# yetanotherco/yet-another-halo2-fork

Hardware: AMD Instinct MI355X
Metric: create_proof wall-seconds at k=22 (BN254/KZG); MSM Mscalar-mul/s at 2^24 (lower is better)
Workload: dtype u32 limbs (BN254 Fr/Fq Montgomery, 256-bit modular integer)

## Files before the change

include/h2g.h:

```cpp
#ifndef H2G_H
#define H2G_H

#include <stddef.h>
#include <stdint.h>

#ifdef __cplusplus
extern "C" {
#endif

enum {
  H2G_OK = 0,
  H2G_ERR_ARG = 1,
  H2G_ERR_DEVICE = 2,
  H2G_ERR_NOMEM = 3,
  H2G_ERR_STATE = 4,
  H2G_ERR_HANDLE = 5,
  H2G_ERR_UNSATISFIED = 6
};

int h2g_abi_version(void);
const char* h2g_last_error(void);

int h2g_init(const int* devices, int ndev);
int h2g_shutdown(void);
// ... 183 lines not shown
int h2g_params_downsize(uint64_t params, uint32_t k, uint64_t* handle);

int h2g_params_write(uint64_t params, int format, uint8_t* out, size_t cap, size_t* len);
int h2g_params_read(const uint8_t* buf, size_t len, int format, uint64_t* handle);

int h2g_keygen(uint64_t params, const h2g_circuit* circuit, uint64_t* pk);
int h2g_pk_free(uint64_t pk);
int h2g_pk_write(uint64_t pk, int format, uint8_t* out, size_t cap, size_t* len);
int h2g_pk_read(uint64_t params, const h2g_circuit* circuit, const uint8_t* buf, size_t len, int format,
                uint64_t* pk);
enum { H2G_COSETS_RESIDENT = 0, H2G_COSETS_STREAMED = 1 };
typedef struct { uint32_t size; uint32_t cosets; } h2g_key_options;
int h2g_keygen_opts(uint64_t params, const h2g_circuit* circuit, const h2g_key_options* opts, uint64_t* pk);
int h2g_pk_read_opts(uint64_t params, const h2g_circuit* circuit, const uint8_t* buf, size_t len, int format,
                     const h2g_key_options* opts, uint64_t* pk);
int h2g_pk_memory(uint64_t pk, uint64_t out[4]);
int h2g_pk_info(uint64_t pk, int32_t info[8]);
int h2g_pk_lookup_sort_hints(uint64_t pk, int32_t* out, int max, int* count);
int h2g_pk_vk_commitments(uint64_t pk, uint64_t* fixed, uint64_t* perm);
int h2g_pk_set_multiopen(uint64_t pk, int scheme);
int h2g_pk_set_transcript(uint64_t pk, int kind);

int h2g_create_proof(uint64_t params, uint64_t pk, const uint64_t* advice, int advice_on_device,
                     const uint64_t* instance, const uint32_t* instance_lens, const uint8_t rng_seed[32],
                     uint32_t vanishing_threads, uint8_t* proof, size_t proof_cap, size_t* proof_len);
typedef struct {
  void* ctx;
  int (*fill)(void* ctx, uint32_t phase, const uint64_t* challenges, uint64_t* advice);
} h2g_witness_source;
int h2g_create_proof_phased(uint64_t params, uint64_t pk, const h2g_witness_source* witness,
                            const uint64_t* instance, const uint32_t* instance_lens, const uint8_t rng_seed[32],
                            uint32_t vanishing_threads, uint8_t* proof, size_t proof_cap, size_t* proof_len);
typedef struct {
  void* ctx;
  int (*fill_bytes)(void* ctx, uint8_t* out, size_t len);
  int (*random_fr)(void* ctx, uint64_t out[4]);
} h2g_rng;
typedef struct {
  void* ctx;
  int (*fill)(void* ctx, uint32_t circuit, uint32_t phase, const uint64_t* challenges, uint64_t* advice);
} h2g_witness_source_multi;
typedef struct {
  uint32_t num_circuits;
  const uint64_t* const* advice;
  int advice_on_device;
  const h2g_witness_source_multi* witness;
  const uint64_t* const* instance;
  const uint32_t* const* instance_lens;
  const h2g_rng* rng;
  const uint8_t* rng_seed;
  uint32_t vanishing_threads;
} h2g_prove_inputs;
int h2g_create_proof_multi(uint64_t params, uint64_t pk, const h2g_prove_inputs* in, uint8_t* proof,
                           size_t proof_cap, size_t* proof_len);
typedef struct { const uint64_t* index; const uint64_t* den; size_t count; } h2g_assigned_dens;
typedef struct {
  void* ctx;
  int (*fill)(void* ctx, uint32_t circuit, uint32_t phase, const uint64_t* challenges, uint64_t* advice,
              h2g_assigned_dens* dens);
} h2g_assigned_source;
int h2g_create_proof_assigned(uint64_t params, uint64_t pk, const h2g_prove_inputs* in,
                              const h2g_assigned_source* source, uint8_t* proof, size_t proof_cap, size_t* proof_len);
int h2g_rng_chacha20(const uint8_t seed[32], h2g_rng* out, uint64_t* handle);
int h2g_rng_free(uint64_t handle);
int h2g_last_challenges(uint64_t* out, int max, int* count);
enum {
  H2G_CHECK_GATE = 1,
  H2G_CHECK_GATE_BLINDING = 2,
  H2G_CHECK_LOOKUP = 3,
  H2G_CHECK_SHUFFLE = 4,
  H2G_CHECK_COPY = 5
};
#define H2G_CHECK_NO_ROW 0xFFFFFFFFu
typedef struct {
  uint32_t kind, index, row, reserved;
} h2g_check_failure;
typedef struct {
  const uint64_t* advice;
  int advice_on_device;
  const uint64_t* instance;
  const uint64_t* challenges;
  const uint8_t* seed;
  const int32_t* copies;
  uint32_t num_copies;
} h2g_check_inputs;
int h2g_check_witness(uint64_t pk, const h2g_check_inputs* in, h2g_check_failure* out, size_t cap, uint64_t* total);

enum { H2G_SELFCHECK_OFF = 0, H2G_SELFCHECK_VERDICT = 1, H2G_SELFCHECK_ARGUMENTS = 2 };
enum {
  H2G_CHECK_PERMUTATION = 6,
  H2G_CHECK_PRODUCT = 7,
  H2G_CHECK_PERMUTED_PAIR = 8,
  H2G_CHECK_UNUSABLE_ROW = 9,
  H2G_CHECK_IDENTITY = 10
};
int h2g_pk_set_self_check(uint64_t pk, int mode);
int h2g_last_self_check(h2g_check_failure* out, size_t cap, uint64_t* total);
int h2g_debug_selfcheck_product_dev(const void* d_z, const void* d_num_a, const void* d_num_b, const void* d_den_a,
                                    const void* d_den_b, const uint64_t beta[4], const uint64_t gamma[4], uint64_t n,
                                    uint64_t u, int max_blocks, h2g_check_failure* out, size_t cap, uint64_t* total);
int h2g_debug_selfcheck_permuted_dev(const void* d_a, const void* d_s, uint64_t u, int max_blocks,
                                     h2g_check_failure* out, size_t cap, uint64_t* total);
int h2g_debug_selfcheck_permutation_dev(const void* d_z, const uint64_t* first, const void* const* d_values,
                                        const void* const* d_sigmas, const uint64_t* delta_pows, int m,
                                        const uint64_t beta[4], const uint64_t gamma[4], const uint64_t omega[4],
                                        uint64_t u, h2g_check_failure* out, size_t cap, uint64_t* total);

int h2g_vk_from_pk(uint64_t pk, uint64_t* vk);
int h2g_vk_read(const h2g_circuit* circuit, const uint8_t* buf, size_t len, int format, uint64_t* vk);
int h2g_vk_write(uint64_t vk, int format, uint8_t* out, size_t cap, size_t* len);
int h2g_vk_free(uint64_t vk);
typedef struct { uint64_t g1[8], g2[16], s_g2[16]; } h2g_verifier_params;
int h2g_params_verifier(uint64_t params, h2g_verifier_params* out);
typedef struct {
  const uint8_t* proof; size_t proof_len;
  uint32_t num_circuits;
  const uint64_t* const* instance;
  const uint32_t* const* instance_lens;
} h2g_verify_item;
enum { H2G_VERIFY_OK = 1, H2G_VERIFY_REJECTED = 0, H2G_VERIFY_MALFORMED = -1 };
int h2g_verify_proof(uint64_t vk, const h2g_verifier_params* vp, int multiopen, int transcript,
                     const h2g_verify_item* item, int32_t* verdict);
int h2g_verify_batch(uint64_t vk, const h2g_verifier_params* vp, int multiopen, int transcript,
                     const h2g_verify_item* items, size_t count, const h2g_rng* rng,
                     int32_t* verdicts, uint64_t stats[4]);
int h2g_verify_stages(double ms[4]);

int h2g_transcript_new_write(int kind, uint64_t* t);
int h2g_transcript_new_read(int kind, const uint8_t* proof, size_t len, uint64_t* t);
int h2g_transcript_common_point(uint64_t t, const uint64_t p[8]);
int h2g_transcript_common_scalar(uint64_t t, const uint64_t s[4]);
int h2g_transcript_write_point(uint64_t t, const uint64_t p[8]);
int h2g_transcript_write_scalar(uint64_t t, const uint64_t s[4]);
int h2g_transcript_read_point(uint64_t t, uint64_t p[8]);
int h2g_transcript_read_scalar(uint64_t t, uint64_t s[4]);
int h2g_transcript_squeeze(uint64_t t, uint64_t c[4]);
int h2g_transcript_bytes(uint64_t t, uint8_t* out, size_t cap, size_t* len);
int h2g_transcript_remaining(uint64_t t, size_t* bytes);
int h2g_transcript_free(uint64_t t);

int h2g_params_commit(uint64_t params, const uint64_t* coeffs, size_t len, uint64_t out[8], int* is_identity);
int h2g_params_commit_lagrange(uint64_t params, const uint64_t* evals, size_t len, uint64_t out[8], int* is_identity);
int h2g_params_commit_dev(uint64_t params, const void* d_coeffs, size_t len, uint64_t out[8], int* is_identity,
                          void* stream);
int h2g_params_commit_lagrange_dev(uint64_t params, const void* d_evals, size_t len, uint64_t out[8],
                                   int* is_identity, void* stream);
int h2g_fr_eval(const uint64_t* poly, size_t len, const uint64_t x[4], uint64_t out[4]);
int h2g_fr_eval_dev(const void* d_poly, size_t len, const uint64_t x[4], uint64_t out[4], void* stream);
int h2g_kate_division(const uint64_t* a, size_t len, const uint64_t b[4], uint64_t* q);
int h2g_kate_division_dev(const void* d_a, size_t len, const uint64_t b[4], void* d_q, void* stream);
int h2g_debug_kate_division_dev(const void* d_a, size_t len, const uint64_t b[4], void* d_q, int accumulate,
                                int tile_s, void* stream);
int h2g_debug_kate_tile_s(size_t len, int* tile_s);

typedef struct { const uint64_t* coeffs; size_t len; int on_device; } h2g_poly_ref;
typedef struct { uint32_t poly; uint32_t reserved; uint64_t point[4]; } h2g_open_query;
int h2g_multiopen_prove(uint64_t params, int scheme, uint64_t transcript, const h2g_poly_ref* polys, size_t npolys,
                        const h2g_open_query* queries, size_t nqueries);
typedef struct { uint32_t commitment; uint32_t reserved; uint64_t point[4]; uint64_t eval[4]; } h2g_verify_query;
int h2g_multiopen_verify(const h2g_verifier_params* vp, int scheme, uint64_t transcript,
                         const uint64_t* commitments, size_t ncommitments,
                         const h2g_verify_query* queries, size_t nqueries, int32_t* verdict, uint64_t lr[16]);

int h2g_pairing_check_batch(const h2g_verifier_params* vp, const uint64_t* lr, size_t count, int32_t* ok);
int h2g_pairing_check_batch_dev(const h2g_verifier_params* vp, const void* d_lr, size_t count,
                                void* d_ok , void* stream);
int h2g_verify_set_isolation(int mode);
int h2g_debug_pairing_values(const h2g_verifier_params* vp, const uint64_t* lr, size_t count,
                             uint64_t* miller, uint64_t* gt);

int h2g_prover_stage_sync(int on);
int h2g_prover_stages(double* ms, int max, int* count);
const char* h2g_prover_stage_name(int i);

typedef struct {
  void* ctx;
  int32_t world;
  int (*launch)(void* ctx, uint64_t seq, int32_t base_set, uint64_t n, const void* d_scalars);
  int (*collect)(void* ctx, uint64_t seq, uint64_t* partials, int32_t* is_identity);
} h2g_shard_transport;
int h2g_set_shard_transport(const h2g_shard_transport* t);
int h2g_params_set_slab(uint64_t params, uint64_t lo, uint64_t hi);
int h2g_params_msm_dev(uint64_t params, int32_t base_set, uint64_t offset, uint64_t n, const void* d_scalars,
                       uint64_t out_affine[8], int32_t* out_is_identity);
int h2g_params_table_bytes(uint64_t params, uint64_t out[4]);
int h2g_memcpy_dtod(void* d_dst, const void* d_src, size_t bytes);

int h2g_comm_unique_id(uint8_t id[256]);
int h2g_comm_init(const uint8_t id[256], int world, int rank);
int h2g_comm_set_timeout(double seconds);
int h2g_comm_set_serve_timeout(double seconds);
int h2g_comm_keepalive(void);
int h2g_comm_install(uint64_t params);
int h2g_comm_serve(uint64_t params, uint64_t* served);
int h2g_comm_stop(void);
int h2g_comm_destroy(void);
int h2g_comm_info(int32_t* rccl_count, int32_t* rccl_rank);

#define H2G_SPMD_WORDS 13
typedef struct {
  void* ctx;
  int32_t world;
  int32_t rank;
  int (*allgather)(void* ctx, uint64_t seq, const uint64_t in[9], uint64_t* out);
  int (*bcast)(void* ctx, void* d_buf, size_t bytes, int root);
  int (*allgather_host)(void* ctx, const void* in, size_t bytes, void* out);
  int (*exchange)(void* ctx, const void* d_send, const size_t* send_bytes, void* d_recv, const size_t* recv_bytes);
} h2g_spmd_transport;
int h2g_set_spmd_transport(const h2g_spmd_transport* t);
typedef int (*h2g_spmd_exchange_post)(void* ctx, const void* d_send, const size_t* send_bytes, void* d_recv,
                                      const size_t* recv_bytes, void* stream, void* done);
typedef int (*h2g_spmd_exchange_wait)(void* ctx, void* done);
int h2g_set_spmd_exchange_async(h2g_spmd_exchange_post post, h2g_spmd_exchange_wait wait);
int h2g_event_wait(void* done);
int h2g_debug_link_delay(void* stream, void* done, double us);
int h2g_spmd_set_weights(const uint32_t* weights, int world);
int h2g_spmd_set_column_owners(int on);
int h2g_spmd_stats(double* out, int max, int reset);
int h2g_comm_spmd_install(int split_subcosets);
int h2g_comm_set_exchange_overlap(int on);
int h2g_comm_spmd_uninstall(void);

#ifdef __cplusplus
}
#endif

#endif
```

yet-another-halo2-fork_amd/csrc/keygen.cpp:

```cpp
#include "prover_state.h"

using namespace h2g;
using namespace h2g::rt;
using namespace h2g::prv;

namespace {
struct CircuitView {
  const h2g_circuit* c;
  const int32_t* node(int i) const { return c->nodes + 4 * i; }
};

int node_degree(const CircuitView& v, int i, std::vector<int>& memo) {
  if (memo[i] >= 0) return memo[i];
  const int32_t* nd = v.node(i);
  int d = 0;
  switch (nd[0]) {
    case OP_CONST:
    case OP_CHALLENGE: d = 0; break;
    case OP_QUERY: d = 1; break;
    case OP_NEG: d = node_degree(v, nd[1], memo); break;
    case OP_SUM: d = std::max(node_degree(v, nd[1], memo), node_degree(v, nd[2], memo)); break;
    default: d = node_degree(v, nd[1], memo) + node_degree(v, nd[2], memo); break;
  }
  return memo[i] = d;
// ... 263 lines not shown
  HIPCHK(hipMemcpy(w->d_perm_v, pv.data(), pv.size() * sizeof(Fr*), hipMemcpyHostToDevice));
  pk.cws.push_back(std::move(w));
  return H2G_OK;
}

int key_options_mode(const h2g_key_options* opts, const char* who, int* mode) {
  *mode = H2G_COSETS_RESIDENT;
  if (!opts) return H2G_OK;
  if (opts->size < sizeof(h2g_key_options)) return fail(H2G_ERR_ARG, std::string(who) + ": key options: bad size");
  if (opts->cosets != H2G_COSETS_RESIDENT && opts->cosets != H2G_COSETS_STREAMED)
    return fail(H2G_ERR_ARG, std::string(who) + ": key options: unknown coset mode");
  *mode = (int)opts->cosets;
  return H2G_OK;
}

int build_pow_table(Pool& pool, const Fr& w, int L, PowTable* t, hipStream_t st) {
  const int bits = (L + 1) / 2;
  const size_t nlo = (size_t)1 << bits, nhi = (size_t)1 << (L - bits > 0 ? L - bits : 0);
  std::vector<Fr> lo(nlo), hi(nhi);
  lo[0] = Fr::one();
  for (size_t i = 1; i < nlo; i++) lo[i] = lo[i - 1] * w;
  const Fr wb = lo[nlo - 1] * w;
  hi[0] = Fr::one();
  for (size_t i = 1; i < nhi; i++) hi[i] = hi[i - 1] * wb;
  Fr *dlo, *dhi;
  PALLOC(pool, dlo, nlo);
  PALLOC(pool, dhi, nhi);
  HIPCHK(hipMemcpyAsync(dlo, lo.data(), nlo * sizeof(Fr), hipMemcpyHostToDevice, st));
  HIPCHK(hipMemcpyAsync(dhi, hi.data(), nhi * sizeof(Fr), hipMemcpyHostToDevice, st));
  HIPCHK(hipStreamSynchronize(st));
  t->lo = dlo;
  t->hi = dhi;
  t->bits = bits;
  return H2G_OK;
}

int cs_host_build(const h2g_circuit* c, CsHost* out) {
  CsHost& cs = *out;
  cs = CsHost{};
  std::string why;
  if (c->num_gates && (!c->gate_roots || !c->nodes)) return fail(H2G_ERR_ARG, "keygen: null gates");
  if (!check_nodes(c, &why)) return fail(H2G_ERR_ARG, "keygen: bad expression graph: " + why);
  if (!c->transcript_repr) return fail(H2G_ERR_ARG, "keygen: null transcript_repr");
  if (c->k > FR_S) return fail(H2G_ERR_ARG, "keygen: k too large");
  const CircuitView cv{c};
  const size_t n = (size_t)1 << c->k;
  cs.k = c->k;
  cs.A = (int)c->num_advice;
  cs.F = (int)c->num_fixed;
  cs.I = (int)c->num_instance;
  cs.P = (int)c->num_perm_columns;
  cs.transcript_repr = fr_from_limbs(c->transcript_repr);
  cs.adv_phase.assign(cs.A, 0);
  if (c->advice_phase)
    for (int i = 0; i < cs.A; i++) cs.adv_phase[i] = c->advice_phase[i];
  cs.ch_phase.assign(c->num_challenges, 0);
  if (c->num_challenges && !c->challenge_phase) return fail(H2G_ERR_ARG, "keygen: null challenge_phase");
  for (uint32_t i = 0; i < c->num_challenges; i++) cs.ch_phase[i] = c->challenge_phase[i];
  cs.max_phase = 0;
  for (int i = 0; i < cs.A; i++) cs.max_phase = std::max(cs.max_phase, (int)cs.adv_phase[i]);
  for (uint8_t ph : cs.ch_phase)
    if ((int)ph > cs.max_phase) return fail(H2G_ERR_ARG, "keygen: challenge phase after the last advice phase");
  if (cs.P && !c->perm_columns) return fail(H2G_ERR_ARG, "keygen: null permutation columns");
  for (int i = 0; i < cs.P; i++) {
    const int t = c->perm_columns[2 * i], ix = c->perm_columns[2 * i + 1];
    const int lim = t == COL_ADVICE ? cs.A : t == COL_FIXED ? cs.F : t == COL_INSTANCE ? cs.I : 0;
    if (ix < 0 || ix >= lim) return fail(H2G_ERR_ARG, "keygen: permutation column out of range");
    cs.perm_cols.emplace_back(t, ix);
  }
  std::vector<int> memo(c->num_nodes, -1);
  const std::vector<ArgRoots> lks = arg_roots(c->num_lookups, c->lookup_sizes, c->lookup_roots);
  const std::vector<ArgRoots> shs = arg_roots(c->num_shuffles, c->shuffle_sizes, c->shuffle_roots);
  cs.NL = (int)lks.size();
  cs.NS = (int)shs.size();
  cs.degree = 3;
  for (uint32_t g = 0; g < c->num_gates; g++) cs.degree = std::max(cs.degree, node_degree(cv, c->gate_roots[g], memo));
  for (const auto& a : lks) {
    int di = 1, dt = 1;
    for (int i = 0; i < a.m; i++) {
      di = std::max(di, node_degree(cv, a.in[i], memo));
      dt = std::max(dt, node_degree(cv, a.other[i], memo));
    }
    cs.degree = std::max(cs.degree, std::max(4, 2 + di + dt));
  }
  for (const auto& a : shs) {
    int di = 1, ds = 1;
    for (int i = 0; i < a.m; i++) {
      di = std::max(di, node_degree(cv, a.in[i], memo));
      ds = std::max(ds, node_degree(cv, a.other[i], memo));
    }
    cs.degree = std::max(cs.degree, 2 + std::max(di, ds));
  }
  for (uint32_t g = 0; g < c->num_gates; g++) collect(cv, c->gate_roots[g], cs);
  for (const auto& a : lks) {
    for (int i = 0; i < a.m; i++) collect(cv, a.in[i], cs);
    for (int i = 0; i < a.m; i++) collect(cv, a.other[i], cs);
  }
  for (const auto& a : shs) {
    for (int i = 0; i < a.m; i++) collect(cv, a.in[i], cs);
    for (int i = 0; i < a.m; i++) collect(cv, a.other[i], cs);
  }
  for (auto& pc : cs.perm_cols)
    add_query(pc.first == COL_ADVICE ? cs.adv_q : (pc.first == COL_FIXED ? cs.fix_q : cs.ins_q),
              Query{pc.first, pc.second, 0});
  int maxq = 1;
  if (cs.A) {
    std::vector<int> cnt(cs.A, 0);
    for (auto& q : cs.adv_q) cnt[q.index]++;
    maxq = *std::max_element(cnt.begin(), cnt.end());
  }
  cs.bf = std::max(3, maxq) + 2;
  if ((int64_t)n < cs.bf + 3) return fail(H2G_ERR_ARG, "keygen: not enough rows available");
  cs.chunk_len = cs.degree - 2;
  cs.nsets = (cs.P + cs.chunk_len - 1) / cs.chunk_len;
  if (c->num_nodes) cs.nodes.assign(c->nodes, c->nodes + 4 * (size_t)c->num_nodes);
  if (c->num_constants && !c->constants) return fail(H2G_ERR_ARG, "keygen: null constants");
  cs.constants.resize(c->num_constants);
  for (uint32_t i = 0; i < c->num_constants; i++) cs.constants[i] = fr_from_limbs(c->constants + 4 * i);
  if (c->num_gates) cs.gate_roots.assign(c->gate_roots, c->gate_roots + c->num_gates);
  for (const auto& a : lks) {
    cs.lk_in.emplace_back(a.in, a.in + a.m);
    cs.lk_tab.emplace_back(a.other, a.other + a.m);
  }
  for (const auto& a : shs) {
    cs.sh_in.emplace_back(a.in, a.in + a.m);
    cs.sh_sh.emplace_back(a.other, a.other + a.m);
  }
  return H2G_OK;
}

int keygen_impl(Device* d, Params& prm, const h2g_circuit* c, ProvingKey& pk, const PkImage* img = nullptr) {
  hipStream_t st = d->stream;
  if (c->k != prm.k) return fail(H2G_ERR_ARG, "keygen: circuit k != params k");
  RCCHK(cs_host_build(c, &pk.cs));
  if (!img && c->num_fixed && !c->fixed_values) return fail(H2G_ERR_ARG, "keygen: null fixed values");
  const CircuitView cv{c};
  const std::vector<ArgRoots> lks = arg_roots(c->num_lookups, c->lookup_sizes, c->lookup_roots);
  const std::vector<ArgRoots> shs = arg_roots(c->num_shuffles, c->shuffle_sizes, c->shuffle_roots);
  pk.device = d->id;
  pk.n = (size_t)1 << pk.cs.k;
  pk.unblinded.assign(pk.cs.A, 0);
  if (c->unblinded)
    for (int i = 0; i < pk.cs.A; i++) pk.unblinded[i] = c->unblinded[i];
  pk.num_consts = (int)c->num_constants;
  RCCHK(domain_init(&pk.dom, (uint32_t)pk.cs.degree, pk.cs.k));
  pk.ext = (size_t)1 << pk.dom.ek;
  pk.rot_scale = 1ull << (pk.dom.ek - pk.cs.k);
  const size_t n = pk.n, ext = pk.ext;
  Pool& pool = pk.pool;
  RCCHK(build_pow_table(pool, pk.dom.omega, (int)pk.cs.k, &pk.om, st));
  RCCHK(build_pow_table(pool, pk.dom.ext_omega, (int)pk.dom.ek, &pk.eo, st));

  auto falloc = [&](Fr** p, size_t cnt) { return pool.get((void**)p, cnt * sizeof(Fr)); };
  pk.scr_len = std::max(n + 64, kate_scratch_len(n) + poly_prefix_scratch_len(n) + 64);
  HIPCHK(falloc(&pk.mod, n));
  HIPCHK(falloc(&pk.pre, n));
  HIPCHK(falloc(&pk.scr, pk.scr_len));
  HIPCHK(falloc(&pk.random_poly, n));
  HIPCHK(falloc(&pk.h_ext, ext));
  HIPCHK(falloc(&pk.h_coeff, ext));
  HIPCHK(falloc(&pk.h_poly, n));
  HIPCHK(falloc(&pk.nx, n));
  HIPCHK(falloc(&pk.q1, n));
  HIPCHK(falloc(&pk.hx, n));
  HIPCHK(falloc(&pk.lx, n));
  HIPCHK(falloc(&pk.small, 4096));
  HIPCHK(falloc(&pk.last_z, 1));
  auto vec_alloc = [&](std::vector<Fr*>& v, int cnt, size_t len) -> hipError_t {
    v.assign(cnt, nullptr);
    for (int i = 0; i < cnt; i++) {
      hipError_t e = falloc(&v[i], len);
      if (e != hipSuccess) return e;
    }
    return hipSuccess;
  };
  HIPCHK(falloc(&pk.one, 1));
  {
    const Fr one = Fr::one();
    HIPCHK(hipMemcpy(pk.one, &one, sizeof(Fr), hipMemcpyHostToDevice));
  }
  if (pk.cs.NL + pk.cs.NS) {
    HIPCHK(falloc(&pk.tmp_a, n));
    HIPCHK(falloc(&pk.tmp_b, n));
  }
  if (pk.cs.NL) {
    PALLOC(pool, pk.ck_a2, n);
    PALLOC(pool, pk.ck_t2, n);
    PALLOC(pool, pk.ck_left, n);
    PALLOC(pool, pk.rep_flag, n);
    PALLOC(pool, pk.left_flag, n);
    PALLOC(pool, pk.rep_rows, n);
    PALLOC(pool, pk.counters, 8);
    pk.lk_hb.assign(pk.cs.NL, 64);
  }

  const bool streamed = pk.cosets != 0;
  const size_t clen = streamed ? n : ext;
  auto image_coset = [&](Fr* resident, const uint8_t* src) -> int {
    Fr* dst = streamed ? pk.h_ext : resident;
    HIPCHK(img->upload(dst, src, ext, st));
    if (streamed && img->bad_raw) HIPCHK(fr_count_unreduced(dst, ext, img->bad_raw, st));
    return H2G_OK;
  };
  if (streamed) HIPCHK(falloc(&pk.h_gather, ext));
  HIPCHK(vec_alloc(pk.fixed_lag, pk.cs.F, n));
  HIPCHK(vec_alloc(pk.fixed_poly, pk.cs.F, n));
  HIPCHK(vec_alloc(pk.fixed_coset, pk.cs.F, clen));
  for (int i = 0; i < pk.cs.F; i++) {
    if (img) {
      HIPCHK(img->upload(pk.fixed_lag[i], img->fixed_lag[i], n, st));
      HIPCHK(img->upload(pk.fixed_poly[i], img->fixed_poly[i], n, st));
      RCCHK(image_coset(pk.fixed_coset[i], img->fixed_coset[i]));
      continue;
    }
    HIPCHK(hipMemcpyAsync(pk.fixed_lag[i], c->fixed_values + 4 * n * i, n * sizeof(Fr), hipMemcpyHostToDevice, st));
    RCCHK(lagrange_to_coeff(d, pk.dom, pk.fixed_lag[i], pk.fixed_poly[i], st));
    if (!streamed) RCCHK(coeff_to_extended(d, pk.dom, pk.fixed_poly[i], pk.fixed_coset[i], st));
  }
  HIPCHK(falloc(&pk.l0, clen));
  HIPCHK(falloc(&pk.l_last, clen));
  HIPCHK(falloc(&pk.l_active, clen));
  if (img) {
    RCCHK(image_coset(pk.l0, img->l0));
    RCCHK(image_coset(pk.l_last, img->l_last));
    RCCHK(image_coset(pk.l_active, img->l_active));
  }
  if (!img || streamed) {
    const Fr one = Fr::one();
    std::vector<Fr> ones(pk.cs.bf, one);
    auto lagrange_unit = [&](size_t row0, int count, Fr* poly, Fr* out) -> int {
      HIPCHK(hipMemsetAsync(pk.pre, 0, n * sizeof(Fr), st));
      HIPCHK(hipMemcpyAsync(pk.pre + row0, ones.data(), count * sizeof(Fr), hipMemcpyHostToDevice, st));
      RCCHK(lagrange_to_coeff(d, pk.dom, pk.pre, poly, st));
      if (out) RCCHK(coeff_to_extended(d, pk.dom, poly, out, st));
      HIPCHK(hipStreamSynchronize(st));
      return H2G_OK;
    };
    if (streamed) {
      HIPCHK(falloc(&pk.l0_poly, n));
      HIPCHK(falloc(&pk.l_last_poly, n));
      HIPCHK(falloc(&pk.l_blind_poly, n));
      RCCHK(lagrange_unit(0, 1, pk.l0_poly, nullptr));
      RCCHK(lagrange_unit(n - pk.cs.bf, pk.cs.bf, pk.l_blind_poly, nullptr));
      RCCHK(lagrange_unit(n - pk.cs.bf - 1, 1, pk.l_last_poly, nullptr));
    } else {
      RCCHK(lagrange_unit(0, 1, pk.mod, pk.l0));
      RCCHK(lagrange_unit(n - pk.cs.bf, pk.cs.bf, pk.mod, pk.h_ext));
      RCCHK(lagrange_unit(n - pk.cs.bf - 1, 1, pk.mod, pk.l_last));
      HIPCHK(poly_binop(POLY_ADD, pk.l_last, pk.h_ext, one, pk.l_active, ext, st));
      HIPCHK(poly_binop(POLY_SUB_CONST, pk.l_active, nullptr, one, pk.l_active, ext, st));
      HIPCHK(poly_binop(POLY_SCALE, pk.l_active, nullptr, fr_neg_one(), pk.l_active, ext, st));
    }
  }
  HIPCHK(vec_alloc(pk.sigma_lag, pk.cs.P, n));
  HIPCHK(vec_alloc(pk.sigma_poly, pk.cs.P, n));
  HIPCHK(vec_alloc(pk.sigma_coset, pk.cs.P, clen));
  if (pk.cs.P && img) {
    for (int i = 0; i < pk.cs.P; i++) {
      HIPCHK(img->upload(pk.sigma_lag[i], img->sigma_lag[i], n, st));
      HIPCHK(img->upload(pk.sigma_poly[i], img->sigma_poly[i], n, st));
      RCCHK(image_coset(pk.sigma_coset[i], img->sigma_coset[i]));
    }
    HIPCHK(hipStreamSynchronize(st));
  } else if (pk.cs.P) {
    const size_t cells = (size_t)pk.cs.P * n;
    std::vector<uint32_t> mcol(cells), mrow(cells), acol(cells), arow(cells);
    std::vector<uint64_t> sizes(cells, 1);
    for (int cI = 0; cI < pk.cs.P; cI++)
      for (size_t r = 0; r < n; r++) {
        mcol[cI * n + r] = acol[cI * n + r] = (uint32_t)cI;
        mrow[cI * n + r] = arow[cI * n + r] = (uint32_t)r;
      }
    auto pos = [&](int t, int ix) -> int {
      for (int i = 0; i < pk.cs.P; i++)
        if (pk.cs.perm_cols[i].first == t && pk.cs.perm_cols[i].second == ix) return i;
      return -1;
    };
    for (uint32_t ci = 0; ci < c->num_copies; ci++) {
      const int32_t* cp = c->copies + 6 * ci;
      const int lc = pos(cp[0], cp[1]), rc = pos(cp[3], cp[4]);
      if (lc < 0 || rc < 0) return fail(H2G_ERR_ARG, "keygen: copy on a column not in the permutation");
      if (cp[2] < 0 || cp[5] < 0 || (size_t)cp[2] >= n || (size_t)cp[5] >= n)
        return fail(H2G_ERR_ARG, "keygen: copy row out of bounds");
      const size_t li = lc * n + cp[2], ri = rc * n + cp[5];
      size_t lcyc = acol[li] * n + arow[li], rcyc = acol[ri] * n + arow[ri];
      if (lcyc == rcyc) continue;
      if (sizes[lcyc] < sizes[rcyc]) std::swap(lcyc, rcyc);
      sizes[lcyc] += sizes[rcyc];
      size_t i = rcyc;
      for (;;) {
        acol[i] = (uint32_t)(lcyc / n);
        arow[i] = (uint32_t)(lcyc % n);
        i = (size_t)mcol[i] * n + mrow[i];
        if (i == rcyc) break;
      }
      std::swap(mcol[li], mcol[ri]);
      std::swap(mrow[li], mrow[ri]);
    }
    std::vector<Fr> dpow(pk.cs.P + 1);
    dpow[0] = Fr::one();
    for (int i = 1; i <= pk.cs.P; i++) dpow[i] = dpow[i - 1] * fr_delta();
    uint32_t *dmc, *dmr;
    Fr* ddp;
    HIPCHK(hipMalloc(&dmc, cells * 4));
    HIPCHK(hipMalloc(&dmr, cells * 4));
    HIPCHK(hipMalloc(&ddp, dpow.size() * sizeof(Fr)));
    HIPCHK(hipMemcpyAsync(dmc, mcol.data(), cells * 4, hipMemcpyHostToDevice, st));
// ... 194 lines not shown
```

yet-another-halo2-fork_amd/csrc/kzg.cpp:

```cpp
#include "multiopen.h"

using namespace h2g;
using namespace h2g::rt;
using namespace h2g::prv;

namespace h2g {
namespace prv {
std::map<uint64_t, std::unique_ptr<TranscriptObj>> g_transcripts;

bool TranscriptObj::read_point(G1Affine* out) {
  if (!read || bytes.size() - pos < 32) return false;
  G1Affine p;
  if (!g1_from_bytes_host(bytes.data() + pos, &p) || p.is_identity()) return false;
  if (!tr.common_point(p)) return false;
  pos += 32;
  *out = p;
  return true;
}
bool TranscriptObj::read_scalar(Fr* out) {
  if (!read || bytes.size() - pos < 32) return false;
  Fr c;
  std::memcpy(c.l, bytes.data() + pos, 32);
  unsigned br = 0;
  for (int i = 0; i < 8; i++) (void)__builtin_subc(c.l[i], FrParams::M[i], br, &br);
// ... 87 lines not shown
  if (len) obj->bytes.assign(proof, proof + len);
  *t = g_next_handle++;
  g_transcripts[*t] = std::move(obj);
  return H2G_OK;
}
int h2g_transcript_free(uint64_t t) {
  std::lock_guard<std::recursive_mutex> lk(g_mu);
  if (!g_transcripts.erase(t)) return fail(H2G_ERR_HANDLE, "unknown transcript");
  return H2G_OK;
}
int h2g_transcript_common_point(uint64_t t, const uint64_t p[8]) {
  NEED_TRANSCRIPT(t);
  G1Affine a;
  if (!p || !point_arg(p, &a)) return fail(H2G_ERR_ARG, "transcript: not a point of the curve, or the identity");
  T->tr.common_point(a);
  return H2G_OK;
}
int h2g_transcript_common_scalar(uint64_t t, const uint64_t s[4]) {
  NEED_TRANSCRIPT(t);
  if (!s || !fr_reduced(fr_from_limbs(s))) return fail(H2G_ERR_ARG, "transcript: scalar not below r");
  T->tr.common_scalar(fr_from_limbs(s));
  return H2G_OK;
}
int h2g_transcript_write_point(uint64_t t, const uint64_t p[8]) {
  NEED_TRANSCRIPT(t);
  if (T->read) return fail(H2G_ERR_ARG, "transcript_write_point: a read-mode transcript");
  G1Affine a;
  if (!p || !point_arg(p, &a))
    return fail(H2G_ERR_ARG, "cannot write points at infinity (or off the curve) to the transcript");
  T->tr.write_point(a);
  return H2G_OK;
}
int h2g_transcript_write_scalar(uint64_t t, const uint64_t s[4]) {
  NEED_TRANSCRIPT(t);
  if (T->read) return fail(H2G_ERR_ARG, "transcript_write_scalar: a read-mode transcript");
  if (!s || !fr_reduced(fr_from_limbs(s))) return fail(H2G_ERR_ARG, "transcript: scalar not below r");
  T->tr.write_scalar(fr_from_limbs(s));
  return H2G_OK;
}
int h2g_transcript_read_point(uint64_t t, uint64_t p[8]) {
  NEED_TRANSCRIPT(t);
  if (!T->read) return fail(H2G_ERR_ARG, "transcript_read_point: a write-mode transcript");
  G1Affine a;
  if (!p || !T->read_point(&a))
    return fail(H2G_ERR_ARG, "transcript_read_point: the bytes end, or no valid encoding of a point other than the identity");
  std::memcpy(p, &a, sizeof(G1Affine));
  return H2G_OK;
}
int h2g_transcript_read_scalar(uint64_t t, uint64_t s[4]) {
  NEED_TRANSCRIPT(t);
  if (!T->read) return fail(H2G_ERR_ARG, "transcript_read_scalar: a write-mode transcript");
  Fr v;
  if (!s || !T->read_scalar(&v)) return fail(H2G_ERR_ARG, "transcript_read_scalar: the bytes end, or a value >= r");
  fr_to_limbs(v, s);
  return H2G_OK;
}
int h2g_transcript_squeeze(uint64_t t, uint64_t c[4]) {
  NEED_TRANSCRIPT(t);
  if (!c) return fail(H2G_ERR_ARG, "transcript_squeeze: null argument");
  fr_to_limbs(T->tr.squeeze(), c);
  return H2G_OK;
}
int h2g_transcript_bytes(uint64_t t, uint8_t* out, size_t cap, size_t* len) {
  NEED_TRANSCRIPT(t);
  if (T->read) return fail(H2G_ERR_ARG, "transcript_bytes: a read-mode transcript");
  if (!len) return fail(H2G_ERR_ARG, "transcript_bytes: null argument");
  *len = T->bytes.size();
  if (!out) return H2G_OK;
  if (cap < T->bytes.size()) return fail(H2G_ERR_ARG, "transcript_bytes: buffer too small");
  if (!T->bytes.empty()) std::memcpy(out, T->bytes.data(), T->bytes.size());
  return H2G_OK;
}
int h2g_transcript_remaining(uint64_t t, size_t* bytes) {
  NEED_TRANSCRIPT(t);
  if (!T->read) return fail(H2G_ERR_ARG, "transcript_remaining: a write-mode transcript");
  if (!bytes) return fail(H2G_ERR_ARG, "transcript_remaining: null argument");
  *bytes = T->bytes.size() - T->pos;
  return H2G_OK;
}

int h2g_params_commit(uint64_t params, const uint64_t* coeffs, size_t len, uint64_t out[8], int* is_identity) {
  return commit_entry(params, SRS_G, coeffs, false, len, out, is_identity, nullptr);
}
int h2g_params_commit_lagrange(uint64_t params, const uint64_t* evals, size_t len, uint64_t out[8], int* is_identity) {
  return commit_entry(params, SRS_LAGRANGE, evals, false, len, out, is_identity, nullptr);
}
int h2g_params_commit_dev(uint64_t params, const void* d_coeffs, size_t len, uint64_t out[8], int* is_identity,
                          void* stream) {
  return commit_entry(params, SRS_G, d_coeffs, true, len, out, is_identity, stream);
}
int h2g_params_commit_lagrange_dev(uint64_t params, const void* d_evals, size_t len, uint64_t out[8],
                                   int* is_identity, void* stream) {
  return commit_entry(params, SRS_LAGRANGE, d_evals, true, len, out, is_identity, stream);
}

int h2g_fr_eval_dev(const void* d_poly, size_t len, const uint64_t x[4], uint64_t out[4], void* stream) {
  NEED_DEV_P();
  if (!x || !out || (len && !d_poly)) return fail(H2G_ERR_ARG, "fr_eval: null argument");
  if ((uintptr_t)d_poly % 16) return fail(H2G_ERR_ARG, "fr_eval: the polynomial must be 16-byte aligned");
  if (len == 0) {
    fr_to_limbs(Fr::zero(), out);
    return H2G_OK;
  }
  hipStream_t st = pick_stream(d, stream);
  const size_t scr = poly_eval_scratch_len(1, len);
  HIPCHK(d->work.ensure(128 + scr * sizeof(Fr)));
  uint8_t* w = d->work.as<uint8_t>();
  const EvalReq rq{(const Fr*)d_poly, (uint64_t)len, fr_from_limbs(x)};
  Fr r;
  HIPCHK(hipMemcpyAsync(w, &rq, sizeof(rq), hipMemcpyHostToDevice, st));
  HIPCHK(poly_eval_batch((const EvalReq*)w, 1, len, (Fr*)(w + 64), (Fr*)(w + 128), st));
  HIPCHK(hipMemcpyAsync(&r, w + 64, sizeof(Fr), hipMemcpyDeviceToHost, st));
  HIPCHK(hipStreamSynchronize(st));
  fr_to_limbs(r, out);
  return H2G_OK;
}
int h2g_fr_eval(const uint64_t* poly, size_t len, const uint64_t x[4], uint64_t out[4]) {
  NEED_DEV_P();
  if (len && !poly) return fail(H2G_ERR_ARG, "fr_eval: null argument");
  HIPCHK(d->a.ensure(len * sizeof(Fr) + 32));
  HIPCHK(hipMemcpyAsync(d->a.p, poly, len * sizeof(Fr), hipMemcpyHostToDevice, d->stream));
  return h2g_fr_eval_dev(d->a.p, len, x, out, nullptr);
}
int h2g_kate_division_dev(const void* d_a, size_t len, const uint64_t b[4], void* d_q, void* stream) {
  NEED_DEV_P();
  if (len == 0) return fail(H2G_ERR_ARG, "kate_division: an empty polynomial");
  if (!d_a || !b || (len > 1 && !d_q)) return fail(H2G_ERR_ARG, "kate_division: null argument");
  if ((uintptr_t)d_a % 16 || (uintptr_t)d_q % 16)
    return fail(H2G_ERR_ARG, "kate_division: device arrays must be 16-byte aligned");
  if (len == 1) return H2G_OK;
  HIPCHK(d->work.ensure(kate_scratch_len(len) * sizeof(Fr) + 32));
  HIPCHK(kate_division((const Fr*)d_a, len, fr_from_limbs(b), (Fr*)d_q, d->work.as<Fr>(), pick_stream(d, stream)));
  return H2G_OK;
}
int h2g_debug_kate_division_dev(const void* d_a, size_t len, const uint64_t b[4], void* d_q, int accumulate,
                                int tile_s, void* stream) {
  NEED_DEV_P();
  if (len == 0) return fail(H2G_ERR_ARG, "kate_division: an empty polynomial");
  if (!d_a || !b || (len > 1 && !d_q)) return fail(H2G_ERR_ARG, "kate_division: null argument");
  if ((uintptr_t)d_a % 16 || (uintptr_t)d_q % 16)
    return fail(H2G_ERR_ARG, "kate_division: device arrays must be 16-byte aligned");
  if (tile_s != 0 && tile_s != 8 && tile_s != 16 && tile_s != 32 && tile_s != 64)
    return fail(H2G_ERR_ARG, "debug_kate_division: tile_s must be 0, 8, 16, 32 or 64");
  if (len == 1) return H2G_OK;
  HIPCHK(d->work.ensure(kate_scratch_len(len) * sizeof(Fr) + 32));
  HIPCHK(kate_division((const Fr*)d_a, len, fr_from_limbs(b), (Fr*)d_q, d->work.as<Fr>(), pick_stream(d, stream),
                       accumulate != 0, tile_s));
  return H2G_OK;
}
int h2g_debug_kate_tile_s(size_t len, int* tile_s) {
  if (len == 0) return fail(H2G_ERR_ARG, "kate_division: an empty polynomial");
  if (!tile_s) return fail(H2G_ERR_ARG, "debug_kate_tile_s: null argument");
  *tile_s = kate_tile_s((uint64_t)len - 1);
  return H2G_OK;
}
int h2g_kate_division(const uint64_t* a, size_t len, const uint64_t b[4], uint64_t* q) {
  NEED_DEV_P();
  if (len == 0) return fail(H2G_ERR_ARG, "kate_division: an empty polynomial");
  if (!a || !b || (len > 1 && !q)) return fail(H2G_ERR_ARG, "kate_division: null argument");
  if (len == 1) return H2G_OK;
  HIPCHK(d->a.ensure(len * sizeof(Fr) + 32));
  HIPCHK(d->b.ensure(len * sizeof(Fr) + 32));
  HIPCHK(hipMemcpyAsync(d->a.p, a, len * sizeof(Fr), hipMemcpyHostToDevice, d->stream));
  RCCHK(h2g_kate_division_dev(d->a.p, len, b, d->b.p, nullptr));
  HIPCHK(hipMemcpyAsync(q, d->b.p, (len - 1) * sizeof(Fr), hipMemcpyDeviceToHost, d->stream));
  HIPCHK(hipStreamSynchronize(d->stream));
  return H2G_OK;
}

int h2g_multiopen_prove(uint64_t params, int scheme, uint64_t transcript, const h2g_poly_ref* polys, size_t npolys,
                        const h2g_open_query* queries, size_t nqueries) {
  NEED_DEV_P();
  Params* ip = find_params(params);
  if (!ip) return fail(H2G_ERR_HANDLE, "unknown params");
  TranscriptObj* T = find_transcript(transcript);
  if (!T) return fail(H2G_ERR_HANDLE, "unknown transcript");
  Params& prm = *ip;
  if (prm.device != d->id) return fail(H2G_ERR_ARG, "multiopen_prove: params live on another device");
  if (scheme != MULTIOPEN_SHPLONK && scheme != MULTIOPEN_GWC)
    return fail(H2G_ERR_ARG, "multiopen_prove: scheme must be 0 (SHPLONK) or 1 (GWC)");
  if (T->read) return fail(H2G_ERR_ARG, "multiopen_prove: a read-mode transcript");
  if (!polys || !queries || npolys == 0 || nqueries == 0)
    return fail(H2G_ERR_ARG, "multiopen_prove: no polynomials or no queries");
  if (npolys > (1u << 24) || nqueries > (1u << 24)) return fail(H2G_ERR_ARG, "multiopen_prove: too many queries");
  const size_t n = prm.n;
  if (n < 2) return fail(H2G_ERR_ARG, "multiopen_prove: params of a single point");
  if (g_spmd.world > 1 || g_shard.world > 1)
    return fail(H2G_ERR_STATE, "multiopen_prove: a shard or SPMD transport is installed");
  for (size_t i = 0; i < npolys; i++) {
    const h2g_poly_ref& p = polys[i];
    if (!p.coeffs || p.len == 0) return fail(H2G_ERR_ARG, "multiopen_prove: polynomial " + std::to_string(i) + " is empty");
    if (p.len > n)
      return fail(H2G_ERR_ARG, "multiopen_prove: polynomial " + std::to_string(i) + " is longer than the params' n");
    if (p.on_device && (uintptr_t)p.coeffs % 16)
      return fail(H2G_ERR_ARG, "multiopen_prove: device polynomial " + std::to_string(i) + " is not 16-byte aligned");
  }
  std::vector<OpenQ> qs(nqueries);
  for (size_t i = 0; i < nqueries; i++) {
    if (queries[i].poly >= npolys)
      return fail(H2G_ERR_ARG, "multiopen_prove: query " + std::to_string(i) + " names an unknown polynomial");
    qs[i] = {(int)queries[i].poly, fr_from_limbs(queries[i].point)};
    if (!fr_reduced(qs[i].pt)) return fail(H2G_ERR_ARG, "multiopen_prove: query " + std::to_string(i) + ": point not below r");
  }
  hipStream_t st = d->stream;
  if (!prm.kzg_ws) prm.kzg_ws = std::make_shared<MultiopenWs>();
  MultiopenWs& ws = *static_cast<MultiopenWs*>(prm.kzg_ws.get());
  if (!ws.nx) {
    PALLOC(ws.pool, ws.nx, n);
    PALLOC(ws.pool, ws.hx, n);
    PALLOC(ws.pool, ws.lx, n);
    PALLOC(ws.pool, ws.q1, n);
    PALLOC(ws.pool, ws.scr, kate_scratch_len(n));
  }
  HIPCHK(ws.small.ensure(nqueries + 1));
  Pool call;
  MsmRingGuard ring_guard{d};
  StreamSyncGuard guard{st};
  std::vector<PolyRef> prs(npolys);
  for (size_t i = 0; i < npolys; i++) {
    const h2g_poly_ref& p = polys[i];
    if (p.on_device) {
      prs[i] = {(const Fr*)p.coeffs, (uint64_t)p.len};
      continue;
    }
    Fr* dp;
    PALLOC(call, dp, p.len);
    HIPCHK(hipMemcpyAsync(dp, p.coeffs, p.len * sizeof(Fr), hipMemcpyHostToDevice, st));
    prs[i] = {dp, (uint64_t)p.len};
  }
  std::vector<OpenQ> keys;
  std::vector<std::vector<int>> of(npolys);
  auto index = [&](int poly, const Fr& pt) -> int {
    for (int i : of[poly])
      if (keys[i].pt == pt) return i;
    return -1;
  };
  for (const OpenQ& q : qs)
    if (index(q.poly, q.pt) < 0) {
      keys.push_back(q);
      of[q.poly].push_back((int)keys.size() - 1);
    }
  const int nreq = (int)keys.size();
  std::vector<Fr> evals(nreq);
  {
    uint64_t max_len = 1;
    std::vector<EvalReq> reqs(nreq);
    for (int i = 0; i < nreq; i++) {
      reqs[i] = EvalReq{prs[keys[i].poly].p, prs[keys[i].poly].len, keys[i].pt};
      max_len = std::max<uint64_t>(max_len, reqs[i].len);
    }
    EvalReq* d_reqs;
    Fr *d_out, *d_scr;
    PALLOC(call, d_reqs, nreq);
    PALLOC(call, d_out, nreq);
    PALLOC(call, d_scr, poly_eval_scratch_len(nreq, max_len));
    HIPCHK(hipMemcpyAsync(d_reqs, reqs.data(), nreq * sizeof(EvalReq), hipMemcpyHostToDevice, st));
    HIPCHK(poly_eval_batch(d_reqs, nreq, max_len, d_out, d_scr, st));
    HIPCHK(hipMemcpyAsync(evals.data(), d_out, nreq * sizeof(Fr), hipMemcpyDeviceToHost, st));
    HIPCHK(hipStreamSynchronize(st));
  }
  TranscriptObj run = *T;
  MultiopenCtx c;
  c.d = d;
  c.prm = &prm;
  c.st = st;
  c.tr = &run.tr;
  c.n = n;
  c.polys = &prs;
  c.queries = &qs;
  c.ev = [&](int poly, const Fr& pt) { return evals[index(poly, pt)]; };
  c.nx = ws.nx, c.hx = ws.hx, c.lx = ws.lx, c.q1 = ws.q1, c.scr = ws.scr, c.small = ws.small.p;
  c.gwc_q = &ws.gwc_q;
  c.pool = &ws.pool;
  c.upload = [st](void* dst, const void* src, size_t bytes) {
    return hipMemcpyAsync(dst, src, bytes, hipMemcpyHostToDevice, st);
  };
  c.sl = Slab{0, n, n};
  RCCHK(scheme == MULTIOPEN_GWC ? multiopen_gwc(c) : multiopen_shplonk(c));
  HIPCHK(hipStreamSynchronize(st));
  *T = run;
  return H2G_OK;
}

}
```

yet-another-halo2-fork_amd/csrc/multiopen.cpp:

```cpp
#include "multiopen.h"

using namespace h2g;
using namespace h2g::rt;
using namespace h2g::prv;

namespace {
std::vector<std::vector<Fr>> lagrange_basis(const std::vector<Fr>& pts) {
  const size_t m = pts.size();
  std::vector<std::vector<Fr>> out(m);
  for (size_t j = 0; j < m; j++) {
    std::vector<Fr> num(1, Fr::one());
    Fr den = Fr::one();
    for (size_t k = 0; k < m; k++) {
      if (k == j) continue;
      std::vector<Fr> nn(num.size() + 1, Fr::zero());
      for (size_t i = 0; i < num.size(); i++) {
        nn[i + 1] = nn[i + 1] + num[i];
        nn[i] = nn[i] - pts[k] * num[i];
      }
      num.swap(nn);
      den = den * (pts[j] - pts[k]);
    }
    const Fr sc = inv(den);
    for (Fr& c : num) c = c * sc;
// ... 49 lines not shown
}
void mark(MultiopenCtx& c, const char* name) {
  if (c.mark) c.mark(name);
}
}

namespace h2g {
namespace prv {

int fr_cmp(const Fr& a, const Fr& b) {
  const Fr ca = to_canonical(a), cb = to_canonical(b);
  for (int i = 7; i >= 0; i--) {
    if (ca.l[i] < cb.l[i]) return -1;
    if (ca.l[i] > cb.l[i]) return 1;
  }
  return 0;
}

int multiopen_gwc(MultiopenCtx& c) {
  Transcript& tr = *c.tr;
  const std::vector<PolyRef>& polys = *c.polys;
  const std::vector<OpenQ>& queries = *c.queries;
  const size_t n = c.n;
  hipStream_t st = c.st;
  const Fr v = tr.squeeze();
  std::vector<char> done(queries.size(), 0);
  std::vector<MsmTicket> tk;
  std::vector<Fr> neg_evb;
  neg_evb.reserve(queries.size());
  StreamSyncGuard evb_guard{st};
  for (size_t i = 0; i < queries.size(); i++) {
    if (done[i]) continue;
    const Fr z = queries[i].pt;
    const size_t g = tk.size();
    if (g >= c.gwc_q->size()) {
      Fr* q;
      PALLOC(*c.pool, q, n);
      c.gwc_q->push_back(q);
    }
    LinTerms t;
    bool first = true;
    Fr vp = Fr::one(), evb = Fr::zero();
    for (size_t j = i; j < queries.size(); j++) {
      if (done[j] || queries[j].pt != z) continue;
      done[j] = 1;
      if (t.k == LIN_MAXT - 1) {
        HIPCHK(lincomb(c.nx, n, t, !first, st));
        first = false;
        t.k = 0;
      }
      t.p[t.k] = polys[queries[j].poly].p;
      t.len[t.k] = polys[queries[j].poly].len;
      t.coef[t.k] = vp;
      t.k++;
      evb = evb + vp * c.ev(queries[j].poly, z);
      vp = vp * v;
    }
    neg_evb.push_back(Fr::zero() - evb);
    HIPCHK(c.upload(c.small + g, &neg_evb.back(), sizeof(Fr)));
    t.p[t.k] = c.small + g;
    t.len[t.k] = 1;
    t.coef[t.k] = Fr::one();
    t.k++;
    HIPCHK(lincomb(c.nx, n, t, !first, st));
    HIPCHK(kate_division(c.nx, n, z, (*c.gwc_q)[g], c.scr, st));
    tk.emplace_back();
    RCCHK(commit_launch(c.d, *c.prm, (*c.gwc_q)[g], n - 1, SRS_G, st, &tk.back()));
  }
  {
    std::vector<MsmTicket*> tl;
    for (auto& t : tk) tl.push_back(&t);
    std::vector<G1Affine> cms(tl.size());
    RCCHK(commit_collect_all(c.d, tl.data(), (int)tl.size(), cms.data()));
    for (const G1Affine& cm : cms) RCCHK(write_point(c, cm));
  }
  HIPCHK(hipStreamSynchronize(st));
  mark(c, "gwc");
  return H2G_OK;
}

int multiopen_shplonk(MultiopenCtx& c) {
  Transcript& tr = *c.tr;
  const std::vector<PolyRef>& polys = *c.polys;
  const std::vector<OpenQ>& queries = *c.queries;
  const size_t n = c.n;
  hipStream_t st = c.st;
  const bool slabs = c.slabs;
  const Slab sl = slabs ? c.sl : Slab{0, n, n};
  std::vector<std::vector<Fr>> corr_stage;
  Fr c0_stage;
  StreamSyncGuard corr_guard{st};
  const Fr sy = tr.squeeze();
  std::vector<Fr> super_pts;
  for (auto& q : queries) {
    bool f = false;
    for (auto& p : super_pts) f = f || p == q.pt;
    if (!f) super_pts.push_back(q.pt);
  }
  std::sort(super_pts.begin(), super_pts.end(), [](const Fr& a, const Fr& b) { return fr_cmp(a, b) < 0; });
  std::vector<int> cm_ids;
  std::vector<std::vector<Fr>> cm_pts;
  for (auto& q : queries) {
    int f = -1;
    for (size_t i = 0; i < cm_ids.size(); i++)
      if (cm_ids[i] == q.poly) f = (int)i;
    if (f < 0) {
      f = (int)cm_ids.size();
      cm_ids.push_back(q.poly);
      cm_pts.emplace_back();
    }
    auto& ps = cm_pts[f];
    if (std::find(ps.begin(), ps.end(), q.pt) == ps.end()) ps.push_back(q.pt);
  }
  for (auto& ps : cm_pts) std::sort(ps.begin(), ps.end(), [](const Fr& a, const Fr& b) { return fr_cmp(a, b) < 0; });
  std::vector<int> rs_of(cm_ids.size()), rs_rep;
  for (size_t ci = 0; ci < cm_ids.size(); ci++) {
    int f = -1;
    for (size_t r = 0; r < rs_rep.size(); r++)
      if (cm_pts[rs_rep[r]] == cm_pts[ci]) f = (int)r;
    if (f < 0) {
      f = (int)rs_rep.size();
      rs_rep.push_back((int)ci);
    }
    rs_of[ci] = f;
  }
  std::vector<std::vector<std::vector<Fr>>> basis(rs_rep.size());
  for (size_t r = 0; r < rs_rep.size(); r++) basis[r] = lagrange_basis(cm_pts[rs_rep[r]]);
  std::vector<std::vector<Fr>> low(cm_ids.size());
  for (size_t ci = 0; ci < cm_ids.size(); ci++) {
    const auto& B = basis[rs_of[ci]];
    const size_t m = cm_pts[ci].size();
    low[ci].assign(m, Fr::zero());
    for (size_t j = 0; j < m; j++) {
      const Fr e = c.ev(cm_ids[ci], cm_pts[ci][j]);
      for (size_t i = 0; i < m; i++) low[ci][i] = low[ci][i] + B[j][i] * e;
    }
  }
  const Fr v = tr.squeeze();
  {
    std::vector<Fr> vpow(rs_rep.size()), ypow(cm_ids.size());
    {
      Fr vp = Fr::one();
      for (size_t r = 0; r < rs_rep.size(); r++) {
        vpow[r] = vp;
        vp = vp * v;
        Fr yp = Fr::one();
        for (size_t ci = 0; ci < cm_ids.size(); ci++)
          if (rs_of[ci] == (int)r) {
            ypow[ci] = yp;
            yp = yp * sy;
          }
      }
    }
    const size_t np = super_pts.size(), cap = sl.hi1 - sl.lo + 1;
    if (slabs) HIPCHK(c.slab_pk->slab_buf.ensure(np * cap));
    auto gbuf = [&](size_t i) { return c.slab_pk->slab_buf.p + i * cap - sl.lo; };
    if (slabs) HIPCHK(hipMemsetAsync(c.hx + sl.lo, 0, (sl.hi1 - sl.lo) * sizeof(Fr), st));
    else HIPCHK(hipMemsetAsync(c.hx, 0, n * sizeof(Fr), st));
    for (size_t pi = 0; pi < np; pi++) {
      const Fr& p = super_pts[pi];
      Fr* gp = slabs ? gbuf(pi) : c.nx;
      std::vector<Fr> alpha(rs_rep.size(), Fr::zero());
      std::vector<char> has(rs_rep.size(), 0);
      size_t ncorr = 0;
      for (size_t r = 0; r < rs_rep.size(); r++) {
        const std::vector<Fr>& pts = cm_pts[rs_rep[r]];
        if (std::find(pts.begin(), pts.end(), p) == pts.end()) continue;
        Fr den = Fr::one();
        for (const Fr& q : pts)
          if (!(q == p)) den = den * (p - q);
        alpha[r] = vpow[r] * inv(den);
        has[r] = 1;
        ncorr = std::max(ncorr, pts.size());
      }
      corr_stage.emplace_back(ncorr, Fr::zero());
      std::vector<Fr>& corr = corr_stage.back();
      LinTerms t;
      bool first = true;
      for (size_t ci = 0; ci < cm_ids.size(); ci++) {
        const int r = rs_of[ci];
        if (!has[r]) continue;
        if (t.k == LIN_MAXT - 1) {
          RCCHK(lincomb_range(gp, sl.lo, sl.hi1, t, !first, st));
          first = false;
          t.k = 0;
        }
        const Fr coef = alpha[r] * ypow[ci];
        t.p[t.k] = polys[cm_ids[ci]].p;
        t.len[t.k] = polys[cm_ids[ci]].len;
        t.coef[t.k] = coef;
        t.k++;
        for (size_t j = 0; j < low[ci].size(); j++) corr[j] = corr[j] + coef * low[ci][j];
      }
      HIPCHK(c.upload(c.small, corr.data(), corr.size() * sizeof(Fr)));
      t.p[t.k] = c.small;
      t.len[t.k] = corr.size();
      t.coef[t.k] = fr_neg_one();
      t.k++;
      RCCHK(lincomb_range(gp, sl.lo, sl.hi1, t, !first, st));
      if (!slabs) HIPCHK(kate_division(c.nx, n, p, c.hx, c.scr, st, true));
    }
    if (slabs) {
      std::vector<Fr> carry;
      RCCHK(slab_carries(c, super_pts, [&](size_t i) { return gbuf(i); }, &carry));
      Fr halo = Fr::zero();
      for (size_t pi = 0; pi < np; pi++) {
        const size_t hq = std::min(sl.hi, n - 1);
        if (hq <= sl.lo) continue;
        HIPCHK(poly_binop(POLY_ADD_CONST, gbuf(pi) + hq, nullptr, super_pts[pi] * carry[pi], gbuf(pi) + hq, 1, st));
        HIPCHK(kate_division(gbuf(pi) + sl.lo, hq - sl.lo + 1, super_pts[pi], c.hx + sl.lo, c.scr, st, true));
        halo = halo + carry[pi];
      }
      if (sl.hi < n) {
        corr_stage.emplace_back(1, halo);
        HIPCHK(c.upload(c.hx + sl.hi, corr_stage.back().data(), sizeof(Fr)));
      }
    }
  }
  {
    G1Affine cm;
    RCCHK(commit(c.d, *c.prm, c.hx, n, SRS_G, &cm, st));
    RCCHK(write_point(c, cm));
  }
  mark(c, "shplonk h");
  const Fr u = tr.squeeze();
  Fr z0 = Fr::one();
  {
    Fr vpow = Fr::one(), c0 = Fr::zero();
    LinTerms t;
    bool first = true;
    auto flush = [&]() -> int {
      RCCHK(lincomb_range(c.lx, sl.lo, sl.hi1, t, !first, st));
      first = false;
      t.k = 0;
      return H2G_OK;
    };
    for (size_t r = 0; r < rs_rep.size(); r++) {
      const std::vector<Fr>& pts = cm_pts[rs_rep[r]];
      Fr zi = Fr::one();
      for (auto& sp : super_pts)
        if (std::find(pts.begin(), pts.end(), sp) == pts.end()) zi = (u - sp) * zi;
      if (r == 0) z0 = zi;
      Fr ypow = Fr::one();
      for (size_t ci = 0; ci < cm_ids.size(); ci++) {
        if (rs_of[ci] != (int)r) continue;
        if (t.k == LIN_MAXT - 2) RCCHK(flush());
        const Fr coef = ypow * zi * vpow;
        t.p[t.k] = polys[cm_ids[ci]].p;
        t.len[t.k] = polys[cm_ids[ci]].len;
        t.coef[t.k] = coef;
        t.k++;
        c0 = c0 - coef * eval_host(low[ci], u);
        ypow = ypow * sy;
      }
      vpow = vpow * v;
    }
    Fr zt = Fr::one();
    for (auto& sp : super_pts) zt = (u - sp) * zt;
    c0_stage = c0;
    HIPCHK(c.upload(c.small, &c0_stage, sizeof(Fr)));
    t.p[t.k] = c.small;
    t.len[t.k] = 1;
    t.coef[t.k] = Fr::one();
    t.k++;
    t.p[t.k] = c.hx;
    t.len[t.k] = n;
    t.coef[t.k] = Fr::zero() - zt;
    t.k++;
    RCCHK(flush());
  }
  if (slabs) {
    std::vector<Fr> carry;
    const std::vector<Fr> pts{u};
    RCCHK(slab_carries(c, pts, [&](size_t) { return c.lx; }, &carry));
    const size_t hq = std::min(sl.hi, n - 1);
    if (hq > sl.lo) {
      HIPCHK(poly_binop(POLY_ADD_CONST, c.lx + hq, nullptr, u * carry[0], c.lx + hq, 1, st));
      HIPCHK(kate_division(c.lx + sl.lo, hq - sl.lo + 1, u, c.q1 + sl.lo, c.scr, st));
      HIPCHK(poly_binop(POLY_SCALE, c.q1 + sl.lo, nullptr, inv(z0), c.q1 + sl.lo, hq - sl.lo, st));
    }
  } else {
    HIPCHK(kate_division(c.lx, n, u, c.q1, c.scr, st));
    HIPCHK(poly_binop(POLY_SCALE, c.q1, nullptr, inv(z0), c.q1, n - 1, st));
  }
  {
    G1Affine cm;
    RCCHK(commit(c.d, *c.prm, c.q1, n - 1, SRS_G, &cm, st));
    RCCHK(write_point(c, cm));
  }
  mark(c, "shplonk final");
  return H2G_OK;
}

void msm_merge(Msm& m) {
  std::stable_sort(m.begin(), m.end(), [](const Term& a, const Term& b) { return a.base < b.base; });
  size_t w = 0;
  for (size_t i = 0; i < m.size(); i++) {
    if (w && m[w - 1].base == m[i].base) m[w - 1].s = m[w - 1].s + m[i].s;
    else m[w++] = m[i];
  }
  m.resize(w);
}

bool multiopen_verify_terms(int scheme, const std::vector<VerifierQ>& queries, MultiopenVerifyIo& io, Msm* left_out,
                            Msm* right_out) {
  Transcript& T = *io.T;
  const std::vector<Fr>& point = io.point;
  const Fr one = Fr::one();
  Msm& left = *left_out;
  Msm& right = *right_out;
  if (scheme == MULTIOPEN_GWC) {
    const Fr v = T.squeeze();
    std::vector<int> group_pt;
    std::vector<std::vector<const VerifierQ*>> groups;
    for (const auto& q : queries) {
      size_t g = 0;
      while (g < group_pt.size() && group_pt[g] != q.pt) g++;
      if (g == group_pt.size()) {
        group_pt.push_back(q.pt);
        groups.emplace_back();
      }
      groups[g].push_back(&q);
    }
    if (io.expect_groups >= 0 && groups.size() != (size_t)io.expect_groups) return false;
    std::vector<uint32_t> ws(groups.size());
    for (auto& w : ws) w = io.read_point();
    const Fr u = T.squeeze();
    if (!io.ok()) return false;
    Fr eval_multi = Fr::zero(), upow = one;
    for (size_t g = 0; g < groups.size(); g++) {
      Fr evb = Fr::zero(), vpow = one;
      for (const VerifierQ* q : groups[g]) {
        io.add_obj(right, q->key, vpow * upow);
        evb = evb + vpow * q->eval;
        vpow = vpow * v;
      }
      eval_multi = eval_multi + upow * evb;
      right.push_back({ws[g], upow * point[group_pt[g]]});
      left.push_back({ws[g], upow});
      upow = upow * u;
    }
    right.push_back({BASE_G1, Fr::zero() - eval_multi});
    return true;
  }
  struct Cm {
    uint32_t key;
    std::vector<int> pts;
    std::vector<Fr> evals;
  };
  std::vector<Cm> cms;
  for (const auto& q : queries) {
    size_t i = 0;
    while (i < cms.size() && cms[i].key != q.key) i++;
    if (i == cms.size()) cms.push_back({q.key, {}, {}});
    Cm& cm = cms[i];
    size_t p = 0;
    while (p < cm.pts.size() && cm.pts[p] < q.pt) p++;
    if (p < cm.pts.size() && cm.pts[p] == q.pt) {
      cm.evals[p] = q.eval;
    } else {
      cm.pts.insert(cm.pts.begin() + p, q.pt);
      cm.evals.insert(cm.evals.begin() + p, q.eval);
    }
  }
  std::vector<std::vector<int>> set_pts;
  std::vector<std::vector<const Cm*>> set_cms;
  for (const auto& cm : cms) {
    size_t s = 0;
    while (s < set_pts.size() && set_pts[s] != cm.pts) s++;
    if (s == set_pts.size()) {
      set_pts.push_back(cm.pts);
      set_cms.emplace_back();
    }
    set_cms[s].push_back(&cm);
  }
  std::vector<int> super;
  for (const auto& q : queries)
    if (std::find(super.begin(), super.end(), q.pt) == super.end()) super.push_back(q.pt);
  const Fr sy = T.squeeze();
  const Fr v = T.squeeze();
  const uint32_t h1 = io.read_point();
  const Fr u = T.squeeze();
  const uint32_t h2 = io.read_point();
  if (!io.ok()) return false;
  Fr z0 = Fr::zero(), z0_diff_inv = Fr::zero(), r_outer = Fr::zero(), vpow = one;
  for (size_t s = 0; s < set_pts.size(); s++) {
    const std::vector<int>& pts_s = set_pts[s];
    Fr z_diff = one;
    for (int p : super)
      if (std::find(pts_s.begin(), pts_s.end(), p) == pts_s.end()) z_diff = z_diff * (u - point[p]);
    if (s == 0) {
      z0 = one;
      for (int p : pts_s) z0 = z0 * (u - point[p]);
      z0_diff_inv = inv(z_diff);
      z_diff = one;
    } else {
      z_diff = z_diff * z0_diff_inv;
    }
    std::vector<Fr> basis(pts_s.size());
    for (size_t j = 0; j < pts_s.size(); j++) {
      Fr num = one, den = one;
      for (size_t k = 0; k < pts_s.size(); k++) {
        if (k == j) continue;
        num = num * (u - point[pts_s[k]]);
        den = den * (point[pts_s[j]] - point[pts_s[k]]);
      }
      basis[j] = num * inv(den);
    }
    Fr r_inner = Fr::zero(), ypow = one;
    const Fr scale = vpow * z_diff;
    for (const Cm* cm : set_cms[s]) {
      Fr ru = Fr::zero();
      for (size_t j = 0; j < pts_s.size(); j++) ru = ru + cm->evals[j] * basis[j];
      r_inner = r_inner + ypow * ru;
      io.add_obj(right, cm->key, ypow * scale);
      ypow = ypow * sy;
    }
    r_outer = r_outer + vpow * r_inner * z_diff;
    vpow = vpow * v;
  }
  right.push_back({BASE_G1, Fr::zero() - r_outer});
  right.push_back({h1, Fr::zero() - z0});
  right.push_back({h2, u});
  left.push_back({h2, one});
  return true;
}

}
}
```

yet-another-halo2-fork_amd/csrc/prover_kernels.h:

```cpp
#pragma once
#include "bn254.h"

namespace h2g {

struct PowTable {
  const Fr* lo = nullptr;
  const Fr* hi = nullptr;
  int bits = 0;
};

static constexpr int PERM_MAXC = 8;
struct PermCols {
  const Fr* v[PERM_MAXC];
  const Fr* sigma[PERM_MAXC];
  Fr beta_delta[PERM_MAXC];
  int m = 0;
};
hipError_t perm_denominators(Fr* out, size_t n, const PermCols& c, const Fr& beta, const Fr& gamma, bool init,
                             hipStream_t st);
hipError_t perm_numerators(Fr* mod, size_t n, const PermCols& c, const Fr& gamma, const PowTable& omega,
                           hipStream_t st, size_t r0 = 0);
hipError_t perm_z_assemble(Fr* z, size_t n, int bf, const Fr* prefix, const Fr* last_z, const Fr* blind_rows,
                           hipStream_t st, size_t lo = 0, size_t hi = ~(size_t)0);

// ... 20 lines not shown
  const EvalLookup* lookups = nullptr;
  const EvalShuffle* shuffles = nullptr;
  const Fr* consts = nullptr;
  const Fr* const* query_col = nullptr;
  const int* query_rot = nullptr;
  int nsets = 0, chunk_len = 0, P = 0;
  const Fr* const* z = nullptr;
  const Fr* const* perm_v = nullptr;
  const Fr* const* sigma = nullptr;
  const Fr* l0 = nullptr;
  const Fr* l_last = nullptr;
  const Fr* l_active = nullptr;
  Fr beta, gamma, y, delta_start, delta;
  PowTable ext_omega;
  uint64_t ext = 0, rot_scale = 0;
  uint64_t row0 = 0, rows = 0;
  int last_rot = 0;
  const Fr* t_evals = nullptr;
  uint64_t t_mask = 0;
  const Fr* acc_in = nullptr;
  int divide = 1;
  Fr* out = nullptr;
};
hipError_t evaluate_h(const EvalHArgs& a, hipStream_t st);

hipError_t subcoset_twist(const Fr* src, Fr* dst, size_t n, const PowTable& eo, uint64_t t, uint64_t ext_mask,
                          hipStream_t st);
hipError_t subcoset_gather(const Fr* full, Fr* out, size_t n, uint64_t t, int e, hipStream_t st);
hipError_t subcoset_scatter(const Fr* subs, Fr* ext, size_t n, int e, hipStream_t st);
struct CopySeg {
  const Fr* src;
  Fr* dst;
  uint64_t len;
};
hipError_t copy_segments(const CopySeg* d_segs, int nseg, uint64_t max_len, hipStream_t st);
static constexpr int COPY_COLS_MAX = 16;
struct ColCopy {
  const Fr* src[COPY_COLS_MAX];
  Fr* dst[COPY_COLS_MAX];
  unsigned long long* sum[COPY_COLS_MAX];
};
hipError_t copy_columns(const ColCopy& b, int m, size_t n, bool sums, hipStream_t st);

static constexpr int PREFIX_DIFF_MAX = 16;
struct PrefixDiff {
  const Fr* a[PREFIX_DIFF_MAX];
  Fr* e[PREFIX_DIFF_MAX];
};
hipError_t prefix_diff(const PrefixDiff& b, int m, size_t n, hipStream_t st);
int evaluate_h_max_slots();
static constexpr int HSLAB_MAX_E = 16;
struct HSlabArgs {
  const Fr* recv = nullptr;
  int idx[HSLAB_MAX_E] = {};
  int E = 0, np = 0;
  uint64_t cnt = 0, n = 0, lo = 0;
  const Fr* coef = nullptr;
  Fr* out = nullptr;
};
hipError_t h_slab_combine(const HSlabArgs& a, hipStream_t st);

struct CompressArgs {
  const int4* prog = nullptr;
  int2 seg = {0, 0};
  int n_slots = 0;
  const Fr* consts = nullptr;
  const Fr* const* load_col = nullptr;
  const int* load_rot = nullptr;
  uint64_t n = 0;
  Fr theta;
  Fr* out = nullptr;
};
hipError_t compress_lagrange(const CompressArgs& a, hipStream_t st);
static constexpr int COMPRESS_BATCH_MAX = 32;
struct CompressBatch {
  const int4* prog = nullptr;
  int n_slots = 0;
  const Fr* consts = nullptr;
  const int* load_rot = nullptr;
  uint64_t n = 0;
  Fr theta;
  int count = 0;
  int2 seg[COMPRESS_BATCH_MAX];
  const Fr* const* load_col[COMPRESS_BATCH_MAX];
  Fr* out[COMPRESS_BATCH_MAX];
};
hipError_t compress_lagrange_batch(const CompressBatch& a, hipStream_t st);

struct CanonKey {
  uint32_t l[8];
};
struct CanonLess {
  __host__ __device__ bool operator()(const CanonKey& a, const CanonKey& b) const {
    for (int i = 7; i >= 0; i--)
      if (a.l[i] != b.l[i]) return a.l[i] < b.l[i];
    return false;
  }
};
hipError_t fr_to_canon(const Fr* in, CanonKey* out, size_t n, hipStream_t st);
static constexpr int LOOKUP_KEYS_BATCH_MAX = 32;
struct LookupKeysBatch {
  size_t n = 0;
  CanonKey* canon = nullptr;
  uint64_t* key = nullptr;
  uint32_t* idx = nullptr;
  uint64_t kmask = 0;
  int kbits = 48;
  int count = 0;
  const Fr* in[LOOKUP_KEYS_BATCH_MAX];
  int s[LOOKUP_KEYS_BATCH_MAX];
  int g[LOOKUP_KEYS_BATCH_MAX];
  unsigned long long* d_or[LOOKUP_KEYS_BATCH_MAX];
};
hipError_t lookup_keys_batch(const LookupKeysBatch& b, hipStream_t st);
hipError_t lookup_keys(const Fr* in, size_t n, int s, CanonKey* canon, uint64_t* key, uint32_t* idx,
                       unsigned long long* d_or, hipStream_t st, int kbits = 64, uint64_t tag = 0);
hipError_t lookup_gather(const CanonKey* canon, const uint32_t* idx, size_t u, CanonKey* out,
                         unsigned long long* unsorted, hipStream_t st);
hipError_t key64_expand(const uint64_t* in, CanonKey* out, size_t n, hipStream_t st);
hipError_t lookup_mark(const CanonKey* a, const CanonKey* t, size_t u, uint8_t* rep_flag, uint8_t* left_flag,
                       uint32_t* fail, hipStream_t st);
hipError_t lookup_assign(const CanonKey* a, const uint8_t* rep_flag, size_t u, Fr* ap, Fr* sp, hipStream_t st);
hipError_t lookup_scatter(const CanonKey* L, const uint32_t* R, const uint32_t* d_nrep, size_t cap, Fr* sp,
                          hipStream_t st);
hipError_t lookup_prod_den(const Fr* ap, const Fr* sp, const Fr& beta, const Fr& gamma, Fr* prod, size_t n,
                           hipStream_t st);
hipError_t lookup_prod_num(const Fr* a, const Fr* s, const Fr& beta, const Fr& gamma, Fr* prod, size_t n,
                           hipStream_t st);
hipError_t shuffle_prod_den(const Fr* s, const Fr& gamma, Fr* prod, size_t n, hipStream_t st);
hipError_t shuffle_prod_num(const Fr* a, const Fr& gamma, Fr* prod, size_t n, hipStream_t st);

struct EvalReq {
  const Fr* poly;
  uint64_t len;
  Fr x;
};
hipError_t poly_eval_batch(const EvalReq* d_reqs, int nreq, uint64_t max_len, Fr* d_out, Fr* scratch,
                           hipStream_t st);
size_t poly_eval_scratch_len(int nreq, uint64_t max_len);

hipError_t kate_division(const Fr* a, uint64_t len, const Fr& b, Fr* q, Fr* scratch, hipStream_t st,
                         bool accumulate = false, int force_s = 0);
size_t kate_scratch_len(uint64_t len);
int kate_tile_s(uint64_t M);

static constexpr int LIN_MAXT = 12;
struct LinTerms {
  const Fr* p[LIN_MAXT];
  uint64_t len[LIN_MAXT];
  Fr coef[LIN_MAXT];
  int k = 0;
};
hipError_t lincomb(Fr* out, uint64_t n, const LinTerms& t, bool accumulate, hipStream_t st);
hipError_t scale_by_dev(Fr* out, const Fr* a, uint64_t n, const Fr* scalar, hipStream_t st);

hipError_t sigma_from_mapping(Fr* sigma, const uint32_t* map_col, const uint32_t* map_row, size_t n,
                              const Fr* delta_pow, const PowTable& omega, hipStream_t st);
hipError_t srs_lagrange_scalars(Fr* out, size_t n, const Fr& s, const Fr& mult, const PowTable& omega, Fr* scratch,
                                hipStream_t st);
hipError_t g1_generator_mul(const Fr* scalars, size_t n, G1Affine* out, hipStream_t st);

hipError_t fr_count_unreduced(const Fr* a, size_t n, uint32_t* bad, hipStream_t st);
hipError_t g1_count_invalid(const G1Affine* p, size_t n, uint32_t* bad, hipStream_t st);

hipError_t g1_compress(const G1Affine* p, size_t n, uint8_t* out, hipStream_t st);
hipError_t g1_decompress(const uint8_t* in, size_t n, G1Affine* out, uint32_t* bad, hipStream_t st);
hipError_t fr_to_repr(const Fr* a, size_t n, Fr* out, hipStream_t st);
hipError_t fr_from_repr(Fr* a, size_t n, uint32_t* bad, hipStream_t st);

}
```

yet-another-halo2-fork_amd/csrc/prover_kernels.hip:

```cpp
#include <algorithm>

#include "f29.h"
#include "fr_io.h"
#include "gate_prog.h"
#include "poly.h"
#include "prover_kernels.h"
#include "transcript.h"

namespace h2g {

static constexpr int KT = 256;

static unsigned grid_1d(size_t n, int per_block = KT) {
  size_t g = (n + per_block - 1) / per_block;
  const size_t cap = 256 * 16;
  return (unsigned)(g < cap ? (g ? g : 1) : cap);
}

__device__ __forceinline__ Fr pw(const PowTable& t, uint64_t i) {
  const uint64_t mask = (1ull << t.bits) - 1;
  return ldf(t.lo + (i & mask)) * ldf(t.hi + (i >> t.bits));
}

__global__ void __launch_bounds__(KT) perm_den_kernel(Fr* __restrict__ out, size_t n, PermCols c, Fr beta, Fr gamma,
// ... 574 lines not shown
  if (base >= rq.len) {
    if (threadIdx.x == 0) part[blockIdx.y * nbmax + blockIdx.x] = Fr::zero();
    return;
  }
  __shared__ Fr pw[EV_L + 1];
  __shared__ F29 x29;
  const int t = threadIdx.x;
  if (t == 0) {
    Fr step = rq.x;
    for (int l = 0; l <= EV_L; l++) {
      pw[l] = step;
      step = step * step;
    }
    x29 = storage_to_f29<FrParams>(pw[EV_L]);
  }
  __syncthreads();
  const uint64_t lo = base + (uint64_t)t;
  const F29 X = x29;
  F29 a29{};
  for (int i = EV_S - 1; i >= 0; i--) {
    const uint64_t j = lo + (uint64_t)i * EV_T;
    a29 = add29(mul29<FrParams>(a29, X), j < rq.len ? raw29(ldf(rq.poly + j)) : F29{});
  }
  sh[t] = f29_to_storage(a29);
  __syncthreads();
#pragma unroll
  for (int l = 0; l < EV_L; l++) {
    const int s = 1 << l;
    if ((t & (2 * s - 1)) == 0) sh[t] = sh[t] + pw[l] * sh[t + s];
    __syncthreads();
  }
  if (t == 0) part[blockIdx.y * nbmax + blockIdx.x] = sh[0];
}

__global__ void __launch_bounds__(EV_T) eval_level2(const EvalReq* __restrict__ reqs, const Fr* __restrict__ part,
                                                    uint64_t nbmax, Fr* __restrict__ out) {
  __shared__ Fr sh[EV_T];
  const EvalReq rq = reqs[blockIdx.x];
  const uint64_t nb = (rq.len + EV_BLK - 1) / EV_BLK;
  const uint64_t per = (nb + EV_T - 1) / EV_T;
  Fr xb = rq.x;
  for (int i = 0; i < EV_LB; i++) xb = xb * xb;
  const Fr* p = part + blockIdx.x * nbmax;
  const uint64_t lo = (uint64_t)threadIdx.x * per;
  Fr acc = Fr::zero();
  for (uint64_t i = per; i-- > 0;) {
    const uint64_t j = lo + i;
    acc = acc * xb + (j < nb ? p[j] : Fr::zero());
  }
  const Fr step = pow_u64(xb, per);
  const Fr r = block_weighted_sum<EV_T>(acc, step, sh);
  if (threadIdx.x == 0) out[blockIdx.x] = r;
}

size_t poly_eval_scratch_len(int nreq, uint64_t max_len) {
  const uint64_t nb = (max_len + EV_BLK - 1) / EV_BLK;
  return (size_t)nreq * (nb ? nb : 1);
}

hipError_t poly_eval_batch(const EvalReq* d_reqs, int nreq, uint64_t max_len, Fr* d_out, Fr* scratch,
                           hipStream_t st) {
  if (nreq == 0) return hipSuccess;
  uint64_t nb = (max_len + EV_BLK - 1) / EV_BLK;
  if (nb == 0) nb = 1;
  hipLaunchKernelGGL(eval_level1, dim3((unsigned)nb, (unsigned)nreq), dim3(EV_T), 0, st, d_reqs, scratch, nb);
  hipLaunchKernelGGL(eval_level2, dim3((unsigned)nreq), dim3(EV_T), 0, st, d_reqs, (const Fr*)scratch, nb, d_out);
  return hipGetLastError();
}

#ifndef H2G_KD_S_MAX
#define H2G_KD_S_MAX 32
#endif
static constexpr int KD_T = 256;
static constexpr int KD_S_MIN = 8;
static constexpr int KD_S_MAX = H2G_KD_S_MAX;
static constexpr uint64_t KD_MIN_BLOCKS = 512;
static constexpr int KD_L = 8;
static_assert((1 << KD_L) == KD_T, "KD_L");
static_assert(KD_S_MAX >= KD_S_MIN && KD_S_MAX <= 64, "KD_S_MAX");

struct KatePow {
  Fr p[KD_L + 1];
};

#ifndef H2G_KD_SUB
#define H2G_KD_SUB 4
#endif
static constexpr int KD_SUB = H2G_KD_SUB;
static constexpr int KD_ROW = 2 * KD_SUB + 1;
struct KateStage {
  uint4 v[KD_T * KD_ROW];
};
template <int KD_S>
__device__ __forceinline__ void kate_stage_load(KateStage& st, const Fr* __restrict__ src, uint64_t tile0, uint64_t M,
                                                int c) {
  constexpr int PER = 2 * KD_SUB;
#pragma unroll
  for (int k = 0; k < PER; k++) {
    const int u = k * KD_T + threadIdx.x;
    const int tt = u / PER, r = u % PER;
    const uint64_t j = tile0 + (uint64_t)tt * KD_S + (uint64_t)KD_SUB * c + (r >> 1);
    st.v[tt * KD_ROW + r] = j < M ? reinterpret_cast<const uint4*>(src + j)[r & 1] : make_uint4(0, 0, 0, 0);
  }
}
template <int KD_S>
__device__ __forceinline__ void kate_stage_store(const KateStage& st, Fr* __restrict__ dst, uint64_t tile0,
                                                 uint64_t M, int c) {
  constexpr int PER = 2 * KD_SUB;
#pragma unroll
  for (int k = 0; k < PER; k++) {
    const int u = k * KD_T + threadIdx.x;
    const int tt = u / PER, r = u % PER;
    const uint64_t j = tile0 + (uint64_t)tt * KD_S + (uint64_t)KD_SUB * c + (r >> 1);
    if (j < M) reinterpret_cast<uint4*>(dst + j)[r & 1] = st.v[tt * KD_ROW + r];
  }
}
__device__ __forceinline__ Fr kate_stage_get(const KateStage& st, int t, int i) {
  const uint4 a = st.v[t * KD_ROW + 2 * i], b = st.v[t * KD_ROW + 2 * i + 1];
  Fr r;
  r.l[0] = a.x, r.l[1] = a.y, r.l[2] = a.z, r.l[3] = a.w;
  r.l[4] = b.x, r.l[5] = b.y, r.l[6] = b.z, r.l[7] = b.w;
  return r;
}
__device__ __forceinline__ void kate_stage_put(KateStage& st, int t, int i, const Fr& v) {
  st.v[t * KD_ROW + 2 * i] = make_uint4(v.l[0], v.l[1], v.l[2], v.l[3]);
  st.v[t * KD_ROW + 2 * i + 1] = make_uint4(v.l[4], v.l[5], v.l[6], v.l[7]);
}

template <int KD_S>
__global__ void __launch_bounds__(KD_T) kate_phase1(const Fr* __restrict__ a1, uint64_t M, Fr b, F29 b29, KatePow pw,
                                                    Fr* __restrict__ tile_val, Fr* __restrict__ thr_val) {
  __shared__ Fr sh[KD_T];
  const int t = threadIdx.x;
  const uint64_t lo = blockIdx.x * (uint64_t)(KD_T * KD_S) + (uint64_t)t * KD_S;
  F29 a29{};
#pragma unroll
  for (int i = KD_S - 1; i >= 0; i--) {
    const uint64_t j = lo + i;
    a29 = add29(mul29<FrParams>(a29, b29), j < M ? raw29(ldf(a1 + j)) : F29{});
  }
  const Fr acc = f29_to_storage(a29);
  stf(thr_val + blockIdx.x * (uint64_t)KD_T + t, acc);
  sh[t] = acc;
  __syncthreads();
#pragma unroll
  for (int l = 0; l < KD_L; l++) {
    const int s = 1 << l;
    if ((t & (2 * s - 1)) == 0) sh[t] = sh[t] + pw.p[l] * sh[t + s];
    __syncthreads();
  }
  if (t == 0) tile_val[blockIdx.x] = sh[0];
}

__global__ void __launch_bounds__(KD_T) kate_phase2(Fr* __restrict__ tile_val, uint64_t ntiles, Fr B) {
  __shared__ Fr shv[KD_T], shw[KD_T];
  const uint64_t per = (ntiles + KD_T - 1) / KD_T;
  const uint64_t lo = (uint64_t)threadIdx.x * per;
  const uint64_t hi = lo + per < ntiles ? lo + per : ntiles;
  Fr val = Fr::zero(), w = Fr::one();
  for (uint64_t i = hi; i-- > lo;) {
    val = val * B + tile_val[i];
    w = w * B;
  }
  Fr cv, cw;
  block_suffix_affine<KD_T>(val, w, shv, shw, &cv, &cw);
  Fr carry = cv;
  for (uint64_t i = hi; i-- > lo;) {
    const Fr v = tile_val[i];
    tile_val[i] = carry;
    carry = v + B * carry;
  }
}

template <int KD_S, bool ACC>
__global__ void __launch_bounds__(KD_T) kate_phase3(const Fr* __restrict__ a1, uint64_t M, Fr b, F29 b29, KatePow pw,
                                                    const Fr* __restrict__ tile_carry,
                                                    const Fr* __restrict__ thr_val, Fr* __restrict__ q) {
  __shared__ Fr sh[KD_T];
  const int t = threadIdx.x;
  const uint64_t g = blockIdx.x * (uint64_t)KD_T + t;
  Fr x = t + 1 < KD_T ? ldf(thr_val + g + 1) : tile_carry[blockIdx.x];
#pragma unroll
  for (int l = 0; l < KD_L; l++) {
    const int s = 1 << l;
    sh[t] = x;
    __syncthreads();
    if (t + s < KD_T) x = x + pw.p[l] * sh[t + s];
    __syncthreads();
  }
  __shared__ KateStage stg;
  KateStage* out = &stg;
  if constexpr (ACC) {
    __shared__ KateStage old;
    out = &old;
  }
  const uint64_t tile0 = blockIdx.x * (uint64_t)(KD_T * KD_S);
  F29 cur = raw29(x);
  for (int c = KD_S / KD_SUB - 1; c >= 0; c--) {
    __syncthreads();
    kate_stage_load<KD_S>(stg, a1, tile0, M, c);
    if (ACC) kate_stage_load<KD_S>(*out, q, tile0, M, c);
    __syncthreads();
#pragma unroll
    for (int i = KD_SUB - 1; i >= 0; i--) {
      cur = add29(raw29(kate_stage_get(stg, t, i)), mul29<FrParams>(cur, b29));
      kate_stage_put(*out, t, i, f29_to_storage(ACC ? add29(raw29(kate_stage_get(*out, t, i)), cur) : cur));
    }
    __syncthreads();
    kate_stage_store<KD_S>(*out, q, tile0, M, c);
  }
}

template <int S>
static void kate_launch(const Fr* a, uint64_t M, const Fr& b, const F29& b29, const KatePow& pw, Fr* tile, Fr* thr,
                        Fr* q, uint64_t nt, hipStream_t st, bool accumulate) {
  hipLaunchKernelGGL(kate_phase1<S>, dim3((unsigned)nt), dim3(KD_T), 0, st, a + 1, M, b, b29, pw, tile, thr);
  hipLaunchKernelGGL(kate_phase2, dim3(1), dim3(KD_T), 0, st, tile, nt, pw.p[KD_L]);
  if (accumulate)
    hipLaunchKernelGGL((kate_phase3<S, true>), dim3((unsigned)nt), dim3(KD_T), 0, st, a + 1, M, b, b29, pw,
                       (const Fr*)tile, (const Fr*)thr, q);
  else
    hipLaunchKernelGGL((kate_phase3<S, false>), dim3((unsigned)nt), dim3(KD_T), 0, st, a + 1, M, b, b29, pw,
                       (const Fr*)tile, (const Fr*)thr, q);
}

size_t kate_scratch_len(uint64_t len) {
  const uint64_t nt = (len + (uint64_t)KD_T * KD_S_MIN - 1) / ((uint64_t)KD_T * KD_S_MIN);
  return (size_t)(nt + 1 + nt * KD_T);
}

int kate_tile_s(uint64_t M) {
  int S = KD_S_MIN;
  while (S < KD_S_MAX && (M + (uint64_t)KD_T * S * 2 - 1) / ((uint64_t)KD_T * S * 2) >= KD_MIN_BLOCKS) S <<= 1;
  return S;
}

hipError_t kate_division(const Fr* a, uint64_t len, const Fr& b, Fr* q, Fr* scratch, hipStream_t st,
                         bool accumulate, int force_s) {
  if (len < 2) return hipSuccess;
  const uint64_t M = len - 1;
  if (force_s && force_s != 8 && force_s != 16 && force_s != 32 && force_s != 64) return hipErrorInvalidValue;
  const int S = force_s ? force_s : kate_tile_s(M);
  const uint64_t tile_len = (uint64_t)KD_T * S;
  const uint64_t nt = (M + tile_len - 1) / tile_len;
  KatePow pw;
  Fr x = b;
  for (int i = 1; i < S; i <<= 1) x = x * x;
  for (int l = 0; l <= KD_L; l++) {
    pw.p[l] = x;
    x = x * x;
  }
  Fr* tile = scratch;
  Fr* thr = scratch + nt + 1;
  const F29 b29 = storage_to_f29<FrParams>(b);
  switch (S) {
    case 8: kate_launch<8>(a, M, b, b29, pw, tile, thr, q, nt, st, accumulate); break;
    case 16: kate_launch<16>(a, M, b, b29, pw, tile, thr, q, nt, st, accumulate); break;
    case 32: kate_launch<32>(a, M, b, b29, pw, tile, thr, q, nt, st, accumulate); break;
    default: kate_launch<64>(a, M, b, b29, pw, tile, thr, q, nt, st, accumulate); break;
  }
  return hipGetLastError();
}

struct LinTerms29 {
  const Fr* p[LIN_MAXT];
  uint64_t len[LIN_MAXT];
  F29 coef[LIN_MAXT];
  int k = 0;
};
__global__ void __launch_bounds__(KT) lincomb29_kernel(Fr* __restrict__ out, uint64_t n, LinTerms29 t, int acc_in) {
  for (uint64_t i = blockIdx.x * (uint64_t)blockDim.x + threadIdx.x; i < n; i += (uint64_t)gridDim.x * blockDim.x) {
    F29 acc = acc_in ? raw29(ldf(out + i)) : F29{};
    int k = 0;
    for (; k + 1 < t.k; k += 2) {
      const F29 a = i < t.len[k] ? raw29(ldf(t.p[k] + i)) : F29{};
      const F29 b = i < t.len[k + 1] ? raw29(ldf(t.p[k + 1] + i)) : F29{};
      acc = add29(acc, mul29x2<FrParams>(a, t.coef[k], b, t.coef[k + 1]));
    }
    if (k < t.k) {
      const F29 a = i < t.len[k] ? raw29(ldf(t.p[k] + i)) : F29{};
      acc = add29(acc, mul29<FrParams>(a, t.coef[k]));
    }
    stf(out + i, pack29<FrParams>(sub_m_if_ge29<FrParams>(reduce29<FrParams>(norm29(acc)))));
  }
}

hipError_t lincomb(Fr* out, uint64_t n, const LinTerms& t, bool accumulate, hipStream_t st) {
  if (n == 0) return hipSuccess;
  LinTerms29 t29;
  t29.k = t.k;
  for (int k = 0; k < t.k; k++) {
    t29.p[k] = t.p[k];
    t29.len[k] = t.len[k];
    t29.coef[k] = storage_to_f29<FrParams>(t.coef[k]);
  }
  hipLaunchKernelGGL(lincomb29_kernel, dim3(grid_1d(n)), dim3(KT), 0, st, out, n, t29, accumulate ? 1 : 0);
  return hipGetLastError();
}

__global__ void __launch_bounds__(KT) scale_dev_kernel(Fr* __restrict__ out, const Fr* __restrict__ a, uint64_t n,
                                                       const Fr* __restrict__ s) {
  const Fr c = ldf(s);
  for (uint64_t i = blockIdx.x * (uint64_t)blockDim.x + threadIdx.x; i < n; i += (uint64_t)gridDim.x * blockDim.x)
    stf(out + i, ldf(a + i) * c);
}

hipError_t scale_by_dev(Fr* out, const Fr* a, uint64_t n, const Fr* scalar, hipStream_t st) {
  if (n == 0) return hipSuccess;
  hipLaunchKernelGGL(scale_dev_kernel, dim3(grid_1d(n)), dim3(KT), 0, st, out, a, n, scalar);
  return hipGetLastError();
}

__global__ void __launch_bounds__(KT) subcoset_twist_kernel(const Fr* __restrict__ src, Fr* __restrict__ dst,
                                                            size_t n, PowTable eo, uint64_t t, uint64_t ext_mask) {
  for (size_t j = blockIdx.x * (size_t)blockDim.x + threadIdx.x; j < n; j += (size_t)gridDim.x * blockDim.x)
    stf(dst + j, ldf(src + j) * pw(eo, (t * j) & ext_mask));
}
hipError_t subcoset_twist(const Fr* src, Fr* dst, size_t n, const PowTable& eo, uint64_t t, uint64_t ext_mask,
                          hipStream_t st) {
  if (n == 0) return hipSuccess;
  hipLaunchKernelGGL(subcoset_twist_kernel, dim3(grid_1d(n)), dim3(KT), 0, st, src, dst, n, eo, t, ext_mask);
  return hipGetLastError();
}
__global__ void __launch_bounds__(KT) subcoset_gather_kernel(const Fr* __restrict__ full, Fr* __restrict__ out,
                                                             size_t n, uint64_t t, int e) {
  for (size_t m = blockIdx.x * (size_t)blockDim.x + threadIdx.x; m < n; m += (size_t)gridDim.x * blockDim.x)
    stf(out + m, ldf(full + t + ((uint64_t)m << e)));
}
hipError_t subcoset_gather(const Fr* full, Fr* out, size_t n, uint64_t t, int e, hipStream_t st) {
  if (n == 0) return hipSuccess;
  hipLaunchKernelGGL(subcoset_gather_kernel, dim3(grid_1d(n)), dim3(KT), 0, st, full, out, n, t, e);
  return hipGetLastError();
}
__global__ void __launch_bounds__(KT) copy_segments_kernel(const CopySeg* __restrict__ segs) {
  const CopySeg g = segs[blockIdx.y];
  for (uint64_t i = blockIdx.x * (uint64_t)blockDim.x + threadIdx.x; i < g.len; i += (uint64_t)gridDim.x * blockDim.x)
    stf(g.dst + i, ldf(g.src + i));
}
hipError_t copy_segments(const CopySeg* d_segs, int nseg, uint64_t max_len, hipStream_t st) {
  if (nseg <= 0 || max_len == 0) return hipSuccess;
  const unsigned gx = (unsigned)std::min<uint64_t>((max_len + KT - 1) / KT, 256);
  for (int s0 = 0; s0 < nseg; s0 += 65535)
    hipLaunchKernelGGL(copy_segments_kernel, dim3(gx, (unsigned)std::min(65535, nseg - s0)), dim3(KT), 0, st,
                       d_segs + s0);
  return hipGetLastError();
}
__device__ __forceinline__ uint64_t fmix64(uint64_t x) {
  x ^= x >> 33;
  x *= 0xff51afd7ed558ccdull;
  x ^= x >> 33;
  x *= 0xc4ceb9fe1a85ec53ull;
  return x ^ (x >> 33);
}
__device__ __forceinline__ uint64_t chunk_mix(size_t i, const uint4& v) {
  uint64_t h = fmix64((uint64_t)i * 0x9e3779b97f4a7c15ull + 0x2545f4914f6cdd1dull);
  h = fmix64(h ^ ((uint64_t)v.x | (uint64_t)v.y << 32));
  return fmix64(h ^ ((uint64_t)v.z | (uint64_t)v.w << 32));
}
template <bool SUM>
__global__ void __launch_bounds__(256) copy_columns_kernel(ColCopy b, size_t n2) {
  const uint4* __restrict__ s = reinterpret_cast<const uint4*>(b.src[blockIdx.y]);
  uint4* __restrict__ d = reinterpret_cast<uint4*>(b.dst[blockIdx.y]);
  uint64_t acc = 0;
  const size_t step = (size_t)gridDim.x * 1024;
  for (size_t i = blockIdx.x * (size_t)1024 + threadIdx.x; i < n2; i += step) {
    uint4 v[4];
#pragma unroll
    for (int k = 0; k < 4; k++)
      if (i + 256 * k < n2) v[k] = s[i + 256 * k];
#pragma unroll
    for (int k = 0; k < 4; k++)
      if (i + 256 * k < n2) {
        if (d) d[i + 256 * k] = v[k];
        if (SUM) acc += chunk_mix(i + 256 * k, v[k]);
      }
  }
  if (SUM) {
    for (int o = 32; o > 0; o >>= 1) acc += __shfl_xor(acc, o, 64);
    __shared__ uint64_t part[4];
    if ((threadIdx.x & 63) == 0) part[threadIdx.x >> 6] = acc;
    __syncthreads();
    if (threadIdx.x == 0 && b.sum[blockIdx.y])
      atomicAdd(b.sum[blockIdx.y], (unsigned long long)(part[0] + part[1] + part[2] + part[3]));
  }
}
hipError_t copy_columns(const ColCopy& b, int m, size_t n, bool sums, hipStream_t st) {
  if (m <= 0 || n == 0) return hipSuccess;
  if (m > COPY_COLS_MAX) return hipErrorInvalidValue;
  const size_t n2 = 2 * n;
  const size_t blocks = std::min<size_t>((n2 + 1023) / 1024, 1024);
  if (sums)
    hipLaunchKernelGGL(copy_columns_kernel<true>, dim3((unsigned)blocks, (unsigned)m), dim3(256), 0, st, b, n2);
  else
    hipLaunchKernelGGL(copy_columns_kernel<false>, dim3((unsigned)blocks, (unsigned)m), dim3(256), 0, st, b, n2);
  return hipGetLastError();
}
__global__ void __launch_bounds__(KT) subcoset_scatter_kernel(const Fr* __restrict__ subs, Fr* __restrict__ ext,
                                                              size_t n, int e) {
  const uint64_t total = (uint64_t)n << e, tmask = (1ull << e) - 1;
  for (uint64_t y = blockIdx.x * (uint64_t)blockDim.x + threadIdx.x; y < total; y += (uint64_t)gridDim.x * blockDim.x)
    stf(ext + y, ldf(subs + (y & tmask) * n + (y >> e)));
}
hipError_t subcoset_scatter(const Fr* subs, Fr* ext, size_t n, int e, hipStream_t st) {
  if (n == 0) return hipSuccess;
  hipLaunchKernelGGL(subcoset_scatter_kernel, dim3(grid_1d((size_t)n << e)), dim3(KT), 0, st, subs, ext, n, e);
  return hipGetLastError();
}

__global__ void __launch_bounds__(KT) h_slab_combine_kernel(HSlabArgs a) {
  for (uint64_t j = blockIdx.x * (uint64_t)blockDim.x + threadIdx.x; j < a.cnt; j += (uint64_t)gridDim.x * blockDim.x) {
    Fr f[HSLAB_MAX_E];
    for (int t = 0; t < a.E; t++) f[t] = ldf(a.recv + (uint64_t)a.idx[t] * a.cnt + j);
    for (int p = 0; p < a.np; p++) {
      Fr acc = Fr::zero();
      for (int t = 0; t < a.E; t++) acc = acc + ldf(a.coef + p * a.E + t) * f[t];
      stf(a.out + (uint64_t)p * a.n + a.lo + j, acc);
    }
  }
}
hipError_t h_slab_combine(const HSlabArgs& a, hipStream_t st) {
  if (a.cnt == 0 || a.np == 0) return hipSuccess;
  hipLaunchKernelGGL(h_slab_combine_kernel, dim3(grid_1d(a.cnt)), dim3(KT), 0, st, a);
  return hipGetLastError();
}

__global__ void __launch_bounds__(KT) sigma_kernel(Fr* __restrict__ sigma, const uint32_t* __restrict__ mc,
                                                   const uint32_t* __restrict__ mr, size_t n,
                                                   const Fr* __restrict__ dp, PowTable om) {
  for (size_t i = blockIdx.x * (size_t)blockDim.x + threadIdx.x; i < n; i += (size_t)gridDim.x * blockDim.x)
    stf(sigma + i, ldf(dp + mc[i]) * pw(om, mr[i]));
}

hipError_t sigma_from_mapping(Fr* sigma, const uint32_t* map_col, const uint32_t* map_row, size_t n,
                              const Fr* delta_pow, const PowTable& omega, hipStream_t st) {
  hipLaunchKernelGGL(sigma_kernel, dim3(grid_1d(n)), dim3(KT), 0, st, sigma, map_col, map_row, n, delta_pow, omega);
  return hipGetLastError();
}

__global__ void __launch_bounds__(KT) lag_den_kernel(Fr* __restrict__ d, size_t n, Fr s, PowTable om) {
  for (size_t i = blockIdx.x * (size_t)blockDim.x + threadIdx.x; i < n; i += (size_t)gridDim.x * blockDim.x)
    stf(d + i, s - pw(om, i));
}
__global__ void __launch_bounds__(KT) lag_num_kernel(Fr* __restrict__ d, size_t n, Fr mult, PowTable om) {
  for (size_t i = blockIdx.x * (size_t)blockDim.x + threadIdx.x; i < n; i += (size_t)gridDim.x * blockDim.x)
    stf(d + i, ldf(d + i) * mult * pw(om, i));
}

hipError_t srs_lagrange_scalars(Fr* out, size_t n, const Fr& s, const Fr& mult, const PowTable& omega, Fr* scratch,
                                hipStream_t st) {
  hipLaunchKernelGGL(lag_den_kernel, dim3(grid_1d(n)), dim3(KT), 0, st, out, n, s, omega);
  hipError_t e = poly_batch_invert(out, n, scratch, st);
  if (e != hipSuccess) return e;
// ... 72 lines not shown
```

yet-another-halo2-fork_amd/h2g.py:

```python
import ctypes
import sys
import os
import re

import numpy as np

PKG = os.path.dirname(os.path.abspath(__file__))
REPO = os.path.dirname(PKG)
LIB_PATH = os.environ.get("H2G_LIB") or os.path.join(PKG, "lib", "libh2g.so")
HEADER = os.path.join(REPO, "include", "h2g.h")

U64P = ctypes.POINTER(ctypes.c_uint64)
VP = ctypes.c_void_p
SZ = ctypes.c_size_t
I32 = ctypes.c_int
U32 = ctypes.c_uint32
U64 = ctypes.c_uint64

OP_ADD, OP_SUB, OP_MUL, OP_SCALE, OP_SUB_CONST, OP_ADD_CONST, OP_AXPY = range(7)

_SIGS = {
    "h2g_abi_version": ([], I32),
    "h2g_last_error": ([], ctypes.c_char_p),
    "h2g_init": ([ctypes.POINTER(I32), I32], I32),
# ... 1 lines not shown
    "h2g_device_count": ([ctypes.POINTER(I32)], I32),
    "h2g_device_mem_info": ([ctypes.POINTER(U64), ctypes.POINTER(U64)], I32),
    "h2g_set_device": ([I32], I32),
    "h2g_msm": ([U64P, U64P, SZ, U64P, ctypes.POINTER(I32)], I32),
    "h2g_msm_coeffs_descriptor": ([U64P, SZ, ctypes.POINTER(U64)], I32),
    "h2g_msm_base_descriptor": ([U64P, SZ, ctypes.POINTER(U64)], I32),
    "h2g_msm_descriptor_free": ([U64], I32),
    "h2g_msm_base_descriptor_dev": ([VP, SZ, I32, ctypes.POINTER(U64)], I32),
    "h2g_msm_with_cached_base_dev": ([VP, SZ, U64, SZ, U64P, ctypes.POINTER(I32), VP], I32),
    "h2g_msm_with_cached_scalars": ([U64, U64P, SZ, U64P, ctypes.POINTER(I32)], I32),
    "h2g_msm_with_cached_base": ([U64P, SZ, U64, SZ, U64P, ctypes.POINTER(I32)], I32),
    "h2g_msm_with_cached_inputs": ([U64, U64, SZ, U64P, ctypes.POINTER(I32)], I32),
    "h2g_msm_dev": ([VP, VP, SZ, VP, VP], I32),
    "h2g_msm_dev_cfg": ([VP, VP, SZ, I32, VP, VP], I32),
    "h2g_msm_dev_host": ([VP, VP, SZ, I32, U64P, ctypes.POINTER(I32), VP], I32),
    "h2g_descriptor_device_ptr": ([U64, ctypes.POINTER(VP), ctypes.POINTER(SZ)], I32),
    "h2g_srs_setup_dev": ([U64P, SZ, VP, VP], I32),
    "h2g_fft": ([U64P, U32, U64P], I32),
    "h2g_fft_dev": ([VP, U32, U64P, VP], I32),
    "h2g_domain_create": ([U32, U32, ctypes.POINTER(U64)], I32),
    "h2g_domain_free": ([U64], I32),
    "h2g_domain_info": ([U64, ctypes.POINTER(U32), ctypes.POINTER(U32), U64P], I32),
    "h2g_lagrange_to_coeff": ([U64, U64P], I32),
    "h2g_lagrange_to_coeff_dev": ([U64, VP, VP], I32),
    "h2g_coeff_to_extended": ([U64, U64P, U64P], I32),
    "h2g_coeff_to_extended_dev": ([U64, VP, VP, VP], I32),
    "h2g_coeff_to_subcoset": ([U64, ctypes.POINTER(VP), I32, U64, ctypes.POINTER(VP)], I32),
    "h2g_coeff_to_subcoset_dev": ([U64, ctypes.POINTER(VP), I32, U64, ctypes.POINTER(VP), VP], I32),
    "h2g_debug_coeff_to_subcoset_unfused_dev": ([U64, ctypes.POINTER(VP), I32, U64, ctypes.POINTER(VP), VP], I32),
    "h2g_extended_to_coeff": ([U64, U64P, U64P], I32),
    "h2g_extended_to_coeff_dev": ([U64, VP, VP, VP], I32),
    "h2g_divide_by_vanishing_poly": ([U64, U64P], I32),
    "h2g_divide_by_vanishing_poly_dev": ([U64, VP, VP], I32),
    "h2g_debug_ntt_plan": ([U32, U64, U64, I32, I32, I32, I32, VP], I32),
    "h2g_debug_msm_plan": ([U64, I32, I32, I32, U32, VP], I32),
    "h2g_debug_limits": ([ctypes.POINTER(ctypes.c_int32), I32, ctypes.POINTER(I32)], I32),
    "h2g_debug_commit_batch_chunk": ([I32, U64, ctypes.POINTER(I32)], I32),
    "h2g_debug_msm_batches_dev": ([U64, SZ, ctypes.POINTER(VP), I32, I32, SZ, U64P, ctypes.POINTER(ctypes.c_int32)],
                                  I32),
    "h2g_fr_op": ([I32, U64P, U64P, U64P, U64P, SZ], I32),
    "h2g_fr_op_dev": ([I32, VP, VP, U64P, VP, SZ, VP], I32),
    "h2g_fr_batch_invert": ([U64P, SZ], I32),
    "h2g_fr_batch_invert_dev": ([VP, SZ, VP], I32),
    "h2g_fr_prefix_product": ([U64P, U64P, SZ], I32),
    "h2g_fr_prefix_product_dev": ([VP, VP, SZ, VP], I32),
    "h2g_u32_exclusive_scan_dev": ([VP, VP, SZ, VP], I32),
    "h2g_dev_alloc": ([SZ, ctypes.POINTER(VP)], I32),
    "h2g_dev_free": ([VP], I32),
    "h2g_memcpy_htod": ([VP, VP, SZ], I32),
    "h2g_memcpy_dtoh": ([VP, VP, SZ], I32),
    "h2g_synchronize": ([], I32),
    "h2g_event_create": ([ctypes.POINTER(VP)], I32),
    "h2g_event_destroy": ([VP], I32),
    "h2g_event_record": ([VP, VP], I32),
    "h2g_event_elapsed_ms": ([VP, VP, ctypes.POINTER(ctypes.c_float)], I32),
    "h2g_g1_add_affine": ([U64P, U64P, U64P], I32),
    "h2g_profile_enable": ([I32], I32),
    "h2g_profile_msm_collect": ([ctypes.POINTER(ctypes.c_float), I32, ctypes.POINTER(I32), ctypes.POINTER(I32)], I32),
    "h2g_profile_msm_entries": ([ctypes.POINTER(U64), ctypes.POINTER(I32)], I32),
    "h2g_profile_box_calibrate": ([ctypes.POINTER(ctypes.c_double), I32], I32),
    "h2g_params_create": ([U32, U64P, U64P, ctypes.POINTER(U64)], I32),
    "h2g_params_setup": ([U32, U64P, ctypes.POINTER(U64)], I32),
    "h2g_params_export": ([U64, U64P, U64P], I32),
    "h2g_params_free": ([U64], I32),
    "h2g_params_g2": ([U64, U64P, U64P], I32),
    "h2g_params_set_g2": ([U64, U64P, U64P], I32),
    "h2g_g1_to_lagrange_dev": ([VP, U32, VP, VP], I32),
    "h2g_g1_to_lagrange": ([U64P, U32, U64P], I32),
    "h2g_params_from_parts": ([U32, U64P, U64P, U64P, U64P, ctypes.POINTER(U64)], I32),
    "h2g_params_downsize": ([U64, U32, ctypes.POINTER(U64)], I32),
    "h2g_params_write": ([U64, I32, VP, SZ, ctypes.POINTER(SZ)], I32),
    "h2g_params_read": ([ctypes.c_char_p, SZ, I32, ctypes.POINTER(U64)], I32),
    "h2g_pk_write": ([U64, I32, VP, SZ, ctypes.POINTER(SZ)], I32),
    "h2g_pk_read": ([U64, VP, ctypes.c_char_p, SZ, I32, ctypes.POINTER(U64)], I32),
    "h2g_keygen": ([U64, VP, ctypes.POINTER(U64)], I32),
    "h2g_keygen_opts": ([U64, VP, VP, ctypes.POINTER(U64)], I32),
    "h2g_pk_read_opts": ([U64, VP, ctypes.c_char_p, SZ, I32, VP, ctypes.POINTER(U64)], I32),
    "h2g_pk_memory": ([U64, ctypes.POINTER(U64)], I32),
    "h2g_pk_free": ([U64], I32),
    "h2g_pk_info": ([U64, ctypes.POINTER(ctypes.c_int32)], I32),
    "h2g_pk_vk_commitments": ([U64, U64P, U64P], I32),
    "h2g_pk_lookup_sort_hints": ([U64, ctypes.POINTER(ctypes.c_int32), I32, ctypes.POINTER(I32)], I32),
    "h2g_pk_set_multiopen": ([U64, I32], I32),
    "h2g_pk_set_transcript": ([U64, I32], I32),
    "h2g_create_proof": ([U64, U64, VP, I32, U64P, ctypes.POINTER(U32), ctypes.c_char_p, U32, ctypes.c_char_p, SZ,
                          ctypes.POINTER(SZ)], I32),
    "h2g_create_proof_phased": ([U64, U64, VP, U64P, ctypes.POINTER(U32), ctypes.c_char_p, U32, ctypes.c_char_p,
                                 SZ, ctypes.POINTER(SZ)], I32),
    "h2g_create_proof_multi": ([U64, U64, VP, ctypes.c_char_p, SZ, ctypes.POINTER(SZ)], I32),
    "h2g_check_witness": ([U64, VP, VP, SZ, ctypes.POINTER(U64)], I32),
    "h2g_last_challenges": ([U64P, I32, ctypes.POINTER(I32)], I32),
    "h2g_prover_stages": ([ctypes.POINTER(ctypes.c_double), I32, ctypes.POINTER(I32)], I32),
    "h2g_prover_stage_name": ([I32], ctypes.c_char_p),
    "h2g_prover_stage_sync": ([I32], I32),
    "h2g_set_shard_transport": ([VP], I32),
    "h2g_params_set_slab": ([U64, U64, U64], I32),
    "h2g_params_msm_dev": ([U64, ctypes.c_int32, U64, U64, VP, U64P, ctypes.POINTER(ctypes.c_int32)], I32),
    "h2g_params_table_bytes": ([U64, U64P], I32),
    "h2g_memcpy_dtod": ([VP, VP, SZ], I32),
    "h2g_comm_unique_id": ([ctypes.c_char_p], I32),
    "h2g_comm_init": ([ctypes.c_char_p, I32, I32], I32),
    "h2g_comm_set_timeout": ([ctypes.c_double], I32),
    "h2g_comm_set_serve_timeout": ([ctypes.c_double], I32),
    "h2g_comm_keepalive": ([], I32),
    "h2g_comm_set_exchange_overlap": ([ctypes.c_int32], I32),
    "h2g_comm_install": ([U64], I32),
    "h2g_comm_serve": ([U64, ctypes.POINTER(U64)], I32),
    "h2g_comm_stop": ([], I32),
    "h2g_comm_destroy": ([], I32),
    "h2g_set_spmd_transport": ([VP], I32),
    "h2g_spmd_set_weights": ([VP, I32], I32),
    "h2g_comm_spmd_install": ([I32], I32),
    "h2g_comm_spmd_uninstall": ([], I32),
    "h2g_spmd_set_column_owners": ([I32], I32),
    "h2g_spmd_stats": ([ctypes.POINTER(ctypes.c_double), I32, I32], I32),
    "h2g_rng_chacha20": ([ctypes.POINTER(ctypes.c_uint8), VP, U64P], I32),
    "h2g_rng_free": ([U64], I32),
    "h2g_comm_info": ([ctypes.POINTER(I32), ctypes.POINTER(I32)], I32),
    "h2g_set_spmd_exchange_async": ([VP, VP], I32),
    "h2g_event_wait": ([VP], I32),
    "h2g_debug_link_delay": ([VP, VP, ctypes.c_double], I32),
    "h2g_msm_segmented_dev": ([VP, SZ, VP, VP, VP, SZ, VP, VP], I32),
    "h2g_msm_segmented": ([U64P, SZ, U64P, VP, VP, SZ, U64P], I32),
    "h2g_vk_from_pk": ([U64, ctypes.POINTER(U64)], I32),
    "h2g_vk_read": ([VP, ctypes.c_char_p, SZ, I32, ctypes.POINTER(U64)], I32),
    "h2g_vk_write": ([U64, I32, VP, SZ, ctypes.POINTER(SZ)], I32),
    "h2g_vk_free": ([U64], I32),
    "h2g_params_verifier": ([U64, VP], I32),
    "h2g_verify_proof": ([U64, VP, I32, I32, VP, ctypes.POINTER(ctypes.c_int32)], I32),
    "h2g_verify_batch": ([U64, VP, I32, I32, VP, SZ, VP, ctypes.POINTER(ctypes.c_int32), U64P], I32),
    "h2g_verify_stages": ([ctypes.POINTER(ctypes.c_double)], I32),
    "h2g_transcript_new_write": ([I32, ctypes.POINTER(U64)], I32),
    "h2g_transcript_new_read": ([I32, ctypes.c_char_p, SZ, ctypes.POINTER(U64)], I32),
    "h2g_transcript_common_point": ([U64, U64P], I32),
    "h2g_transcript_common_scalar": ([U64, U64P], I32),
    "h2g_transcript_write_point": ([U64, U64P], I32),
    "h2g_transcript_write_scalar": ([U64, U64P], I32),
    "h2g_transcript_read_point": ([U64, U64P], I32),
    "h2g_transcript_read_scalar": ([U64, U64P], I32),
    "h2g_transcript_squeeze": ([U64, U64P], I32),
    "h2g_transcript_bytes": ([U64, VP, SZ, ctypes.POINTER(SZ)], I32),
    "h2g_transcript_remaining": ([U64, ctypes.POINTER(SZ)], I32),
    "h2g_transcript_free": ([U64], I32),
    "h2g_params_commit": ([U64, U64P, SZ, U64P, ctypes.POINTER(I32)], I32),
    "h2g_params_commit_lagrange": ([U64, U64P, SZ, U64P, ctypes.POINTER(I32)], I32),
    "h2g_params_commit_dev": ([U64, VP, SZ, U64P, ctypes.POINTER(I32), VP], I32),
    "h2g_params_commit_lagrange_dev": ([U64, VP, SZ, U64P, ctypes.POINTER(I32), VP], I32),
    "h2g_fr_eval": ([U64P, SZ, U64P, U64P], I32),
    "h2g_fr_eval_dev": ([VP, SZ, U64P, U64P, VP], I32),
    "h2g_kate_division": ([U64P, SZ, U64P, U64P], I32),
    "h2g_kate_division_dev": ([VP, SZ, U64P, VP, VP], I32),
    "h2g_debug_kate_division_dev": ([VP, SZ, U64P, VP, I32, I32, VP], I32),
    "h2g_debug_kate_tile_s": ([SZ, ctypes.POINTER(I32)], I32),
    "h2g_multiopen_prove": ([U64, I32, U64, VP, SZ, VP, SZ], I32),
    "h2g_multiopen_verify": ([VP, I32, U64, U64P, SZ, VP, SZ, ctypes.POINTER(ctypes.c_int32), U64P], I32),
    "h2g_pairing_check_batch": ([VP, U64P, SZ, ctypes.POINTER(ctypes.c_int32)], I32),
    "h2g_pairing_check_batch_dev": ([VP, VP, SZ, VP, VP], I32),
    "h2g_verify_set_isolation": ([I32], I32),
    "h2g_debug_pairing_values": ([VP, U64P, SZ, U64P, U64P], I32),
    "h2g_assigned_to_fr": ([U64P, SZ, U64P, U64P, SZ, U64P], I32),
    "h2g_assigned_to_fr_dev": ([VP, SZ, VP, VP, SZ, VP, VP], I32),
    "h2g_debug_assigned_per": ([SZ, ctypes.POINTER(I32)], I32),
    "h2g_debug_assigned_to_fr_dev": ([VP, SZ, VP, VP, SZ, VP, I32, VP], I32),
    "h2g_create_proof_assigned": ([U64, U64, VP, VP, ctypes.c_char_p, SZ, ctypes.POINTER(SZ)], I32),
    "h2g_pk_set_self_check": ([U64, I32], I32),
    "h2g_last_self_check": ([VP, SZ, ctypes.POINTER(U64)], I32),
    "h2g_debug_selfcheck_product_dev": ([VP, VP, VP, VP, VP, U64P, U64P, U64, U64, I32, VP, SZ,
                                         ctypes.POINTER(U64)], I32),
    "h2g_debug_selfcheck_permuted_dev": ([VP, VP, U64, I32, VP, SZ, ctypes.POINTER(U64)], I32),
    "h2g_debug_selfcheck_permutation_dev": ([VP, U64P, ctypes.POINTER(VP), ctypes.POINTER(VP), U64P, I32, U64P, U64P,
                                             U64P, U64, VP, SZ, ctypes.POINTER(U64)], I32),
}

TRANSCRIPTS = {"blake2b": 0, "keccak256": 1}
MSM_PHASES = ("partition_coarse", "partition_fine", "bucket_bounds", "accumulate", "bucket_fixup", "reduce")

_lib = None


class H2GError(RuntimeError):

    def __init__(self, msg, code=None, failures=(), total=0):
        super().__init__(msg)
        self.code = code
        self.failures = list(failures)
        self.total = total


class UnsatisfiedError(H2GError):
    """H2G_ERR_UNSATISFIED: the prover's self-check refused a witness that does not satisfy the
    circuit (ProvingKey.set_self_check); no proof was written"""


def header_symbols():
    text = open(HEADER).read()
    return sorted(set(re.findall(r"\b(?:int|const char\*)\s+(h2g_\w+)\s*\(", text)))


def lib():
    global _lib
    if _lib is None:
        if not os.path.exists(LIB_PATH):
            raise H2GError(f"{LIB_PATH} not built: run __graft_entry__.build() "
                           "(yet-another-halo2-fork_amd/build_lib.py)")
        L = ctypes.CDLL(LIB_PATH)
        for name, (args, res) in _SIGS.items():
            if os.environ.get("H2G_LIB") and not hasattr(L, name):
                continue
            f = getattr(L, name)
            f.argtypes = args
            f.restype = res
        _lib = L
    return _lib


ERR_ARG, ERR_DEVICE, ERR_NOMEM, ERR_STATE, ERR_HANDLE, ERR_UNSATISFIED = 1, 2, 3, 4, 5, 6


def check(rc):
    if rc != 0:
        raise H2GError(f"h2g error {rc}: {lib().h2g_last_error().decode()}", code=rc)


def check_proof(rc):
    if rc == 0:
        return
    msg = f"h2g error {rc}: {lib().h2g_last_error().decode()}"
    try:
        total, recs = last_self_check()
    except (H2GError, AttributeError):
        total, recs = 0, []
    raise (UnsatisfiedError if rc == ERR_UNSATISFIED else H2GError)(msg, code=rc, failures=recs, total=total)


def p64(a):
    if a is None:
        return None
    assert a.dtype == np.uint64 and a.flags["C_CONTIGUOUS"], "need C-contiguous uint64"
    return a.ctypes.data_as(U64P)


_inited = False


def init(devices=None):
    global _inited
    tm = sys.modules.get("torch")
    if tm is not None and tm.cuda.device_count() > 0:
        tm.cuda.init()
    if devices:
        arr = (I32 * len(devices))(*devices)
        check(lib().h2g_init(arr, len(devices)))
    else:
        check(lib().h2g_init(None, 0))
    _inited = True


def shutdown():
    global _inited
    check(lib().h2g_shutdown())
    _inited = False


def msm(scalars, bases):
    sc = np.ascontiguousarray(scalars, dtype=np.uint64)
    bs = np.ascontiguousarray(bases, dtype=np.uint64)
    assert sc.shape[0] == bs.shape[0]
    out = np.zeros(8, dtype=np.uint64)
    ident = I32(0)
    check(lib().h2g_msm(p64(sc), p64(bs), sc.shape[0], p64(out), ctypes.byref(ident)))
    return out


def base_descriptor(bases):
    h = U64(0)
    bs = np.ascontiguousarray(bases, dtype=np.uint64)
    check(lib().h2g_msm_base_descriptor(p64(bs), bs.shape[0], ctypes.byref(h)))
    return h.value


def coeffs_descriptor(scalars):
    h = U64(0)
    sc = np.ascontiguousarray(scalars, dtype=np.uint64)
    check(lib().h2g_msm_coeffs_descriptor(p64(sc), sc.shape[0], ctypes.byref(h)))
    return h.value


def base_descriptor_dev(d_bases, n, window_bits=0):
    h = U64()
    check(lib().h2g_msm_base_descriptor_dev(VP(d_bases), n, window_bits, ctypes.byref(h)))
    return h.value


def msm_with_cached_base_dev(d_scalars, n, base_handle, offset=0, stream=None):
    out = np.zeros(8, dtype=np.uint64)
    is_id = I32()
    check(lib().h2g_msm_with_cached_base_dev(VP(d_scalars), n, base_handle, offset, p64(out), ctypes.byref(is_id),
                                             VP(stream) if stream else None))
    return out


def descriptor_free(h):
    check(lib().h2g_msm_descriptor_free(h))


def msm_with_cached_base(scalars, base_handle, offset=0):
# ... 1044 lines not shown
        check(lib().h2g_transcript_squeeze(self.handle, p64(out)))
        return out

    def bytes(self):
        n = SZ()
        check(lib().h2g_transcript_bytes(self.handle, None, 0, ctypes.byref(n)))
        buf = ctypes.create_string_buffer(max(n.value, 1))
        check(lib().h2g_transcript_bytes(self.handle, ctypes.cast(buf, VP), n.value, ctypes.byref(n)))
        return buf.raw[: n.value]

    def remaining(self):
        n = SZ()
        check(lib().h2g_transcript_remaining(self.handle, ctypes.byref(n)))
        return n.value

    def close(self):
        if self.handle:
            lib().h2g_transcript_free(self.handle)
            self.handle = 0


class PolyRef(ctypes.Structure):
    _fields_ = [("coeffs", VP), ("len", SZ), ("on_device", I32)]


class OpenQuery(ctypes.Structure):
    _fields_ = [("poly", U32), ("reserved", U32), ("point", U64 * 4)]


class VerifyQuery(ctypes.Structure):
    _fields_ = [("commitment", U32), ("reserved", U32), ("point", U64 * 4), ("eval", U64 * 4)]


def _limbs4(v):
    a = np.ascontiguousarray(v, dtype=np.uint64).reshape(4)
    return (U64 * 4)(*[int(t) for t in a])


def _commit(fn_host, fn_dev, handle, vals, dev_len, stream):
    out = np.zeros(8, dtype=np.uint64)
    ident = I32(0)
    if dev_len is not None:
        check(fn_dev(handle, VP(vals), dev_len, p64(out), ctypes.byref(ident), VP(stream) if stream else None))
    else:
        a = np.ascontiguousarray(vals, dtype=np.uint64).reshape(-1, 4)
        check(fn_host(handle, p64(a) if a.size else None, len(a), p64(out), ctypes.byref(ident)))
    return out


def _params_commit(self, coeffs, dev_len=None, stream=None):
    return _commit(lib().h2g_params_commit, lib().h2g_params_commit_dev, self.handle, coeffs, dev_len, stream)


def _params_commit_lagrange(self, evals, dev_len=None, stream=None):
    return _commit(lib().h2g_params_commit_lagrange, lib().h2g_params_commit_lagrange_dev, self.handle, evals,
                   dev_len, stream)


def _params_multiopen_prove(self, transcript, polys, queries, scheme="shplonk"):
    keep = []
    refs = (PolyRef * max(len(polys), 1))()
    for i, p in enumerate(polys):
        if isinstance(p, tuple):
            refs[i].coeffs, refs[i].len, refs[i].on_device = p[0], p[1], 1
        else:
            a = np.ascontiguousarray(p, dtype=np.uint64).reshape(-1, 4)
            keep.append(a)
            refs[i].coeffs, refs[i].len, refs[i].on_device = (a.ctypes.data if a.size else None), len(a), 0
    qs = (OpenQuery * max(len(queries), 1))()
    for i, (poly, pt) in enumerate(queries):
        qs[i].poly = poly
        qs[i].point = _limbs4(pt)
    check(lib().h2g_multiopen_prove(self.handle, MULTIOPEN[scheme], transcript.handle, refs, len(polys), qs,
                                    len(queries)))
    del keep


def multiopen_verify(vp, transcript, commitments, queries, scheme="shplonk"):
    cm = np.ascontiguousarray(commitments, dtype=np.uint64).reshape(-1, 8)
    qs = (VerifyQuery * max(len(queries), 1))()
    for i, (c, pt, ev) in enumerate(queries):
        qs[i].commitment = c
        qs[i].point = _limbs4(pt)
        qs[i].eval = _limbs4(ev)
    verdict = ctypes.c_int32(-2)
    lr = np.zeros((2, 8), dtype=np.uint64)
    check(lib().h2g_multiopen_verify(ctypes.byref(vp), MULTIOPEN[scheme], transcript.handle,
                                     p64(cm) if cm.size else None, len(cm), qs, len(queries),
                                     ctypes.byref(verdict), p64(lr)))
    return verdict.value, (lr if verdict.value != VERIFY_MALFORMED else None)


def pairing_check_batch(vp, lr, dev_count=None, d_ok=None, stream=None):
    if dev_count is not None:
        check(lib().h2g_pairing_check_batch_dev(ctypes.byref(vp), VP(lr), dev_count, VP(d_ok),
                                                VP(stream) if stream else None))
        return None
    a = np.ascontiguousarray(lr, dtype=np.uint64).reshape(-1, 16)
    ok = np.zeros(len(a), dtype=np.int32)
    check(lib().h2g_pairing_check_batch(ctypes.byref(vp), p64(a) if a.size else None, len(a),
                                        ok.ctypes.data_as(ctypes.POINTER(ctypes.c_int32))))
    return ok


def verify_set_isolation(mode):
    check(lib().h2g_verify_set_isolation(mode))


def debug_pairing_values(vp, lr, miller=True, gt=True):
    a = np.ascontiguousarray(lr, dtype=np.uint64).reshape(-1, 16)
    m = np.zeros((len(a), 6, 2, 4), dtype=np.uint64) if miller else None
    g = np.zeros((len(a), 6, 2, 4), dtype=np.uint64) if gt else None
    check(lib().h2g_debug_pairing_values(ctypes.byref(vp), p64(a) if a.size else None, len(a),
                                         p64(m) if m is not None and m.size else None,
                                         p64(g) if g is not None and g.size else None))
    return m, g


def fr_eval(poly, x, dev_len=None, stream=None):
    out = np.zeros(4, dtype=np.uint64)
    xs = np.ascontiguousarray(x, dtype=np.uint64)
    if dev_len is not None:
        check(lib().h2g_fr_eval_dev(VP(poly), dev_len, p64(xs), p64(out), VP(stream) if stream else None))
    else:
        a = np.ascontiguousarray(poly, dtype=np.uint64).reshape(-1, 4)
        check(lib().h2g_fr_eval(p64(a) if a.size else None, len(a), p64(xs), p64(out)))
    return out


def kate_division(a, b):
    a = np.ascontiguousarray(a, dtype=np.uint64).reshape(-1, 4)
    q = np.zeros((max(len(a) - 1, 0), 4), dtype=np.uint64)
    check(lib().h2g_kate_division(p64(a) if a.size else None, len(a), p64(np.ascontiguousarray(b, dtype=np.uint64)),
                                  p64(q) if q.size else None))
    return q


def kate_division_dev(d_a, n, b, d_q, stream=None):
    check(lib().h2g_kate_division_dev(VP(d_a), n, p64(np.ascontiguousarray(b, dtype=np.uint64)), VP(d_q),
                                      VP(stream) if stream else None))


def debug_kate_division_dev(d_a, n, b, d_q, accumulate=False, tile_s=0, stream=None):
    check(lib().h2g_debug_kate_division_dev(VP(d_a), n, p64(np.ascontiguousarray(b, dtype=np.uint64)), VP(d_q),
                                            int(bool(accumulate)), tile_s, VP(stream) if stream else None))


def debug_kate_tile_s(n):
    s = I32(0)
    check(lib().h2g_debug_kate_tile_s(n, ctypes.byref(s)))
    return s.value


def msm_segmented(bases, scalars, seg_off, index=None):
    bs = np.ascontiguousarray(bases, dtype=np.uint64).reshape(-1, 8)
    sc = np.ascontiguousarray(scalars, dtype=np.uint64).reshape(-1, 4)
    off = np.ascontiguousarray(seg_off, dtype=np.uint32)
    ix = None if index is None else np.ascontiguousarray(index, dtype=np.uint32)
    nseg = len(off) - 1
    out = np.zeros((max(nseg, 1), 8), dtype=np.uint64)
    check(lib().h2g_msm_segmented(p64(bs) if bs.size else None, len(bs), p64(sc) if sc.size else None,
                                  ix.ctypes.data_as(VP) if ix is not None and ix.size else None,
                                  off.ctypes.data_as(VP), nseg, p64(out)))
    return out[:nseg]


def msm_segmented_dev(d_bases, nbases, d_scalars, d_index, d_seg_off, nseg, d_out, stream=None):
    check(lib().h2g_msm_segmented_dev(VP(d_bases), nbases, VP(d_scalars), VP(d_index) if d_index else None,
                                      VP(d_seg_off), nseg, VP(d_out), VP(stream) if stream else None))


def g1_to_lagrange(g):
    g = np.ascontiguousarray(g, dtype=np.uint64).reshape(-1, 8)
    k = len(g).bit_length() - 1
    if len(g) != 1 << k:
        raise ValueError("g1_to_lagrange: the number of points must be a power of two")
    out = np.zeros_like(g)
    check(lib().h2g_g1_to_lagrange(p64(g), k, p64(out)))
    return out


def g1_to_lagrange_dev(d_g, k, d_out, stream=None):
    check(lib().h2g_g1_to_lagrange_dev(VP(d_g), k, VP(d_out), VP(stream) if stream else None))


SHARD_LAUNCH = ctypes.CFUNCTYPE(ctypes.c_int, VP, U64, ctypes.c_int32, U64, VP)
SHARD_COLLECT = ctypes.CFUNCTYPE(ctypes.c_int, VP, U64, U64P, ctypes.POINTER(ctypes.c_int32))


class ShardTransport(ctypes.Structure):
    _fields_ = [("ctx", VP), ("world", ctypes.c_int32), ("launch", SHARD_LAUNCH), ("collect", SHARD_COLLECT)]


_transport_keep = None


def set_shard_transport(world, launch=None, collect=None):
    global _transport_keep
    if world <= 1:
        check(lib().h2g_set_shard_transport(None))
        _transport_keep = None
        return

    def _launch(ctx, seq, base_set, n, d_scalars):
        try:
            launch(int(seq), int(base_set), int(n), int(d_scalars or 0))
            return 0
        except Exception as e:
            _transport_keep[-1].append(e)
            return 1

    def _collect(ctx, seq, partials, ids):
        try:
            parts = collect(int(seq))
            assert len(parts) == world - 1
            for i, (pt, is_id) in enumerate(parts):
                pt = np.ascontiguousarray(pt, dtype=np.uint64).reshape(8)
                for j in range(8):
                    partials[8 * i + j] = int(pt[j])
                ids[i] = 1 if is_id else 0
            return 0
        except Exception as e:
            _transport_keep[-1].append(e)
            return 1

    cl, cc = SHARD_LAUNCH(_launch), SHARD_COLLECT(_collect)
    t = ShardTransport(None, world, cl, cc)
    _transport_keep = (t, cl, cc, [])
    check(lib().h2g_set_shard_transport(ctypes.byref(t)))


def transport_errors():
    if _transport_keep is None:
        return []
    errs = list(_transport_keep[-1])
    _transport_keep[-1].clear()
    return errs


SPMD_WORDS = 13
_spmd_world = 1
SPMD_ALLGATHER = ctypes.CFUNCTYPE(ctypes.c_int, VP, U64, U64P, U64P)
SPMD_BCAST = ctypes.CFUNCTYPE(ctypes.c_int, VP, VP, SZ, ctypes.c_int)
SPMD_ALLGATHER_HOST = ctypes.CFUNCTYPE(ctypes.c_int, VP, VP, SZ, VP)
SPMD_EXCHANGE = ctypes.CFUNCTYPE(ctypes.c_int, VP, VP, ctypes.POINTER(SZ), VP, ctypes.POINTER(SZ))


class SpmdTransport(ctypes.Structure):
    _fields_ = [("ctx", VP), ("world", ctypes.c_int32), ("rank", ctypes.c_int32), ("allgather", SPMD_ALLGATHER),
                ("bcast", SPMD_BCAST), ("allgather_host", SPMD_ALLGATHER_HOST), ("exchange", SPMD_EXCHANGE)]


def set_spmd_transport(world, rank=0, allgather=None, bcast=None, allgather_host=None, exchange=None):
    global _transport_keep, _spmd_world, _xasync_keep
    _xasync_keep = None
    if world <= 1:
        check(lib().h2g_set_spmd_transport(None))
        _transport_keep = None
        return
    _spmd_world = world

    def _ag(ctx, seq, mine, out):
        try:
            got = np.ascontiguousarray(allgather(int(seq), np.ctypeslib.as_array(mine, shape=(SPMD_WORDS,)).copy()),
                                       dtype=np.uint64).reshape(world * SPMD_WORDS)
            ctypes.memmove(out, got.ctypes.data, world * SPMD_WORDS * 8)
            return 0
        except Exception as e:
            _transport_keep[-1].append(e)
            return 1

    def _bc(ctx, d_ptr, nbytes, root):
        try:
            bcast(int(d_ptr or 0), int(nbytes), int(root))
            return 0
        except Exception as e:
            _transport_keep[-1].append(e)
            return 1

    def _agh(ctx, d_in, nbytes, d_out):
        try:
            parts = allgather_host(ctypes.string_at(d_in, nbytes))
            if len(parts) != world or any(len(p) != nbytes for p in parts):
                raise ValueError("allgather_host: world x bytes expected")
            ctypes.memmove(d_out, b"".join(bytes(p) for p in parts), world * nbytes)
            return 0
        except Exception as e:
            _transport_keep[-1].append(e)
            return 1

    def _ex(ctx, d_send, sbytes, d_recv, rbytes):
        try:
            exchange(int(d_send or 0), [int(sbytes[i]) for i in range(world)], int(d_recv or 0),
                     [int(rbytes[i]) for i in range(world)])
            return 0
        except Exception as e:
            _transport_keep[-1].append(e)
            return 1

    cb = SPMD_ALLGATHER(_ag)
    cbb = SPMD_BCAST(_bc) if bcast is not None else ctypes.cast(None, SPMD_BCAST)
    cbh = SPMD_ALLGATHER_HOST(_agh) if allgather_host is not None else ctypes.cast(None, SPMD_ALLGATHER_HOST)
    cbx = SPMD_EXCHANGE(_ex) if exchange is not None else ctypes.cast(None, SPMD_EXCHANGE)
    t = SpmdTransport(None, world, rank, cb, cbb, cbh, cbx)
    _transport_keep = (t, cb, cbb, cbh, cbx, [])
    check(lib().h2g_set_spmd_transport(ctypes.byref(t)))
# ... 185 lines not shown
```

Measured before the change: 0.07295.

## Batch SHPLONK linear combinations and Kate divisions across up to four points

In the non-slab multiopen path, the per-point linear combinations are replaced by one multi-output lincomb kernel that reads each committed polynomial once and produces up to four outputs. A multi-dividend Kate division then divides all of those outputs in a single three-phase launch that accumulates into the quotient. The final linearisation folds the z0 inverse scaling into the coefficients, which removes a separate scale pass. This cuts repeated global-memory reads of the source polynomials and the number of launches, at the cost of larger scratch buffers, extra per-point buffers and larger kernel argument tables.

```diff
diff --git a/include/h2g.h b/include/h2g.h
--- a/include/h2g.h
+++ b/include/h2g.h
@@ -359,6 +359,11 @@
 int h2g_debug_kate_division_dev(const void* d_a, size_t len, const uint64_t b[4], void* d_q, int accumulate,
                                 int tile_s, void* stream);
 int h2g_debug_kate_tile_s(size_t len, int* tile_s);
+int h2g_debug_lincomb_multi_limits(int* max_outputs, int* max_terms);
+int h2g_debug_lincomb_multi_dev(const void* const* d_terms, const uint64_t* lens, int nterms, const uint64_t* coef,
+                                void* const* d_outs, int nout, size_t n, void* stream);
+int h2g_debug_kate_division_multi_dev(const void* const* d_a, const uint64_t* points, int npoints, size_t len,
+                                      void* d_q, int accumulate, int tile_s, void* stream);
 
 typedef struct { const uint64_t* coeffs; size_t len; int on_device; } h2g_poly_ref;
 typedef struct { uint32_t poly; uint32_t reserved; uint64_t point[4]; } h2g_open_query;
diff --git a/yet-another-halo2-fork_amd/csrc/keygen.cpp b/yet-another-halo2-fork_amd/csrc/keygen.cpp
--- a/yet-another-halo2-fork_amd/csrc/keygen.cpp
+++ b/yet-another-halo2-fork_amd/csrc/keygen.cpp
@@ -439,7 +439,8 @@
   RCCHK(build_pow_table(pool, pk.dom.ext_omega, (int)pk.dom.ek, &pk.eo, st));
 
   auto falloc = [&](Fr** p, size_t cnt) { return pool.get((void**)p, cnt * sizeof(Fr)); };
-  pk.scr_len = std::max(n + 64, kate_scratch_len(n) + poly_prefix_scratch_len(n) + 64);
+  pk.scr_len = std::max({n + 64, kate_scratch_len(n) + poly_prefix_scratch_len(n) + 64,
+                         (size_t)LIN_MAXO * kate_scratch_len(n)});
   HIPCHK(falloc(&pk.mod, n));
   HIPCHK(falloc(&pk.pre, n));
   HIPCHK(falloc(&pk.scr, pk.scr_len));
diff --git a/yet-another-halo2-fork_amd/csrc/kzg.cpp b/yet-another-halo2-fork_amd/csrc/kzg.cpp
--- a/yet-another-halo2-fork_amd/csrc/kzg.cpp
+++ b/yet-another-halo2-fork_amd/csrc/kzg.cpp
@@ -263,6 +263,72 @@
   if (len == 0) return fail(H2G_ERR_ARG, "kate_division: an empty polynomial");
   if (!tile_s) return fail(H2G_ERR_ARG, "debug_kate_tile_s: null argument");
   *tile_s = kate_tile_s((uint64_t)len - 1);
+  return H2G_OK;
+}
+int h2g_debug_lincomb_multi_limits(int* max_outputs, int* max_terms) {
+  if (!max_outputs || !max_terms) return fail(H2G_ERR_ARG, "debug_lincomb_multi_limits: null argument");
+  *max_outputs = LIN_MAXO;
+  *max_terms = LINM_MAXT;
+  return H2G_OK;
+}
+
+int h2g_debug_lincomb_multi_dev(const void* const* d_terms, const uint64_t* lens, int nterms, const uint64_t* coef,
+                                void* const* d_outs, int nout, size_t n, void* stream) {
+  NEED_DEV_P();
+  if (nterms < 0 || nout < 1 || nterms > 4096 || nout > 4096)
+    return fail(H2G_ERR_ARG, "debug_lincomb_multi: term or output count out of range");
+  if (!d_outs || (nterms && (!d_terms || !lens || !coef))) return fail(H2G_ERR_ARG, "debug_lincomb_multi: null argument");
+  std::vector<LinTerm> terms(nterms);
+  std::vector<Fr> cf((size_t)nout * nterms);
+  const size_t bytes = n * sizeof(Fr);
+  for (int o = 0; o < nout; o++) {
+    const uintptr_t a = (uintptr_t)d_outs[o];
+    if (n && (!a || a % 16)) return fail(H2G_ERR_ARG, "debug_lincomb_multi: outputs must be 16-byte aligned");
+    for (int o2 = 0; o2 < o; o2++) {
+      const uintptr_t b = (uintptr_t)d_outs[o2];
+      if (a < b + bytes && b < a + bytes) return fail(H2G_ERR_ARG, "debug_lincomb_multi: outputs overlap");
+    }
+  }
+  for (int k = 0; k < nterms; k++) {
+    const uintptr_t p = (uintptr_t)d_terms[k];
+    if (lens[k] && (!p || p % 16)) return fail(H2G_ERR_ARG, "debug_lincomb_multi: terms must be 16-byte aligned");
+    for (int o = 0; o < nout; o++) {
+      const uintptr_t a = (uintptr_t)d_outs[o];
+      if (lens[k] && a < p + lens[k] * sizeof(Fr) && p < a + bytes)
+        return fail(H2G_ERR_ARG, "debug_lincomb_multi: an output overlaps a term");
+      cf[(size_t)o * nterms + k] = fr_from_limbs(coef + ((size_t)o * nterms + k) * 4);
+      if (!fr_reduced(cf[(size_t)o * nterms + k])) return fail(H2G_ERR_ARG, "debug_lincomb_multi: coefficient not below r");
+    }
+    terms[k] = {(const Fr*)d_terms[k], lens[k]};
+  }
+  HIPCHK(lincomb_multi((Fr* const*)d_outs, nout, n, terms.data(), nterms, cf.data(), pick_stream(d, stream)));
+  return H2G_OK;
+}
+
+int h2g_debug_kate_division_multi_dev(const void* const* d_a, const uint64_t* points, int npoints, size_t len,
+                                      void* d_q, int accumulate, int tile_s, void* stream) {
+  NEED_DEV_P();
+  if (len == 0) return fail(H2G_ERR_ARG, "kate_division_multi: an empty polynomial");
+  if (npoints < 1 || npoints > LIN_MAXO) return fail(H2G_ERR_ARG, "kate_division_multi: 1 .. LIN_MAXO dividends");
+  if (!d_a || !points || (len > 1 && !d_q)) return fail(H2G_ERR_ARG, "kate_division_multi: null argument");
+  if (tile_s != 0 && tile_s != 8 && tile_s != 16 && tile_s != 32 && tile_s != 64)
+    return fail(H2G_ERR_ARG, "debug_kate_division_multi: tile_s must be 0, 8, 16, 32 or 64");
+  if ((uintptr_t)d_q % 16) return fail(H2G_ERR_ARG, "kate_division_multi: device arrays must be 16-byte aligned");
+  Fr b[LIN_MAXO];
+  const Fr* a[LIN_MAXO];
+  for (int p = 0; p < npoints; p++) {
+    const uintptr_t x = (uintptr_t)d_a[p], q = (uintptr_t)d_q;
+    if (!x || x % 16) return fail(H2G_ERR_ARG, "kate_division_multi: device arrays must be 16-byte aligned");
+    if (q < x + len * sizeof(Fr) && x < q + (len - 1) * sizeof(Fr))
+      return fail(H2G_ERR_ARG, "kate_division_multi: the quotient overlaps a dividend");
+    b[p] = fr_from_limbs(points + 4 * p);
+    if (!fr_reduced(b[p])) return fail(H2G_ERR_ARG, "kate_division_multi: point not below r");
+    a[p] = (const Fr*)d_a[p];
+  }
+  if (len == 1) return H2G_OK;
+  HIPCHK(d->work.ensure((size_t)npoints * kate_scratch_len(len) * sizeof(Fr) + 32));
+  HIPCHK(kate_division_multi(a, b, npoints, len, (Fr*)d_q, d->work.as<Fr>(), pick_stream(d, stream), accumulate != 0,
+                             tile_s));
   return H2G_OK;
 }
 int h2g_kate_division(const uint64_t* a, size_t len, const uint64_t b[4], uint64_t* q) {
@@ -321,9 +387,9 @@
     PALLOC(ws.pool, ws.hx, n);
     PALLOC(ws.pool, ws.lx, n);
     PALLOC(ws.pool, ws.q1, n);
-    PALLOC(ws.pool, ws.scr, kate_scratch_len(n));
-  }
-  HIPCHK(ws.small.ensure(nqueries + 1));
+    PALLOC(ws.pool, ws.scr, LIN_MAXO * kate_scratch_len(n));
+  }
+  HIPCHK(ws.small.ensure(LIN_MAXO * (nqueries + 1)));
   Pool call;
   MsmRingGuard ring_guard{d};
   StreamSyncGuard guard{st};
diff --git a/yet-another-halo2-fork_amd/csrc/multiopen.cpp b/yet-another-halo2-fork_amd/csrc/multiopen.cpp
--- a/yet-another-halo2-fork_amd/csrc/multiopen.cpp
+++ b/yet-another-halo2-fork_amd/csrc/multiopen.cpp
@@ -225,19 +225,15 @@
           }
       }
     }
-    const size_t np = super_pts.size(), cap = sl.hi1 - sl.lo + 1;
-    if (slabs) HIPCHK(c.slab_pk->slab_buf.ensure(np * cap));
-    auto gbuf = [&](size_t i) { return c.slab_pk->slab_buf.p + i * cap - sl.lo; };
-    if (slabs) HIPCHK(hipMemsetAsync(c.hx + sl.lo, 0, (sl.hi1 - sl.lo) * sizeof(Fr), st));
-    else HIPCHK(hipMemsetAsync(c.hx, 0, n * sizeof(Fr), st));
-    for (size_t pi = 0; pi < np; pi++) {
-      const Fr& p = super_pts[pi];
-      Fr* gp = slabs ? gbuf(pi) : c.nx;
-      std::vector<Fr> alpha(rs_rep.size(), Fr::zero());
-      std::vector<char> has(rs_rep.size(), 0);
+    const size_t np = super_pts.size(), ncm = cm_ids.size();
+    std::vector<Fr> alpha(rs_rep.size());
+    std::vector<char> has(rs_rep.size());
+    auto alpha_of = [&](const Fr& p) -> size_t {
       size_t ncorr = 0;
       for (size_t r = 0; r < rs_rep.size(); r++) {
         const std::vector<Fr>& pts = cm_pts[rs_rep[r]];
+        alpha[r] = Fr::zero();
+        has[r] = 0;
         if (std::find(pts.begin(), pts.end(), p) == pts.end()) continue;
         Fr den = Fr::one();
         for (const Fr& q : pts)
@@ -246,34 +242,83 @@
         has[r] = 1;
         ncorr = std::max(ncorr, pts.size());
       }
-      corr_stage.emplace_back(ncorr, Fr::zero());
-      std::vector<Fr>& corr = corr_stage.back();
-      LinTerms t;
-      bool first = true;
-      for (size_t ci = 0; ci < cm_ids.size(); ci++) {
-        const int r = rs_of[ci];
-        if (!has[r]) continue;
-        if (t.k == LIN_MAXT - 1) {
-          RCCHK(lincomb_range(gp, sl.lo, sl.hi1, t, !first, st));
-          first = false;
-          t.k = 0;
+      return ncorr;
+    };
+    if (!slabs) {
+      std::vector<Fr*> gbufs{c.nx, c.lx, c.q1};
+      while (gbufs.size() < std::min<size_t>(np, LIN_MAXO)) {
+        const size_t g = gbufs.size() - 3;
+        if (g >= c.gwc_q->size()) {
+          Fr* q;
+          PALLOC(*c.pool, q, n);
+          c.gwc_q->push_back(q);
         }
-        const Fr coef = alpha[r] * ypow[ci];
-        t.p[t.k] = polys[cm_ids[ci]].p;
-        t.len[t.k] = polys[cm_ids[ci]].len;
-        t.coef[t.k] = coef;
+        gbufs.push_back((*c.gwc_q)[g]);
+      }
+      HIPCHK(hipMemsetAsync(c.hx + n - 1, 0, sizeof(Fr), st));
+      for (size_t p0 = 0; p0 < np; p0 += LIN_MAXO) {
+        const size_t P = std::min<size_t>(LIN_MAXO, np - p0), nt = ncm + P;
+        std::vector<LinTerm> terms(nt);
+        std::vector<Fr> coef(P * nt, Fr::zero());
+        for (size_t ci = 0; ci < ncm; ci++) terms[ci] = {polys[cm_ids[ci]].p, polys[cm_ids[ci]].len};
+        std::vector<size_t> corr_off(P + 1, 0);
+        std::vector<std::vector<Fr>> corr(P);
+        for (size_t j = 0; j < P; j++) {
+          corr[j].assign(alpha_of(super_pts[p0 + j]), Fr::zero());
+          for (size_t ci = 0; ci < ncm; ci++) {
+            if (!has[rs_of[ci]]) continue;
+            const Fr cf = alpha[rs_of[ci]] * ypow[ci];
+            coef[j * nt + ci] = cf;
+            for (size_t i = 0; i < low[ci].size(); i++) corr[j][i] = corr[j][i] + cf * low[ci][i];
+          }
+          corr_off[j + 1] = corr_off[j] + corr[j].size();
+          coef[j * nt + ncm + j] = fr_neg_one();
+        }
+        corr_stage.emplace_back();
+        std::vector<Fr>& flat = corr_stage.back();
+        for (size_t j = 0; j < P; j++) {
+          flat.insert(flat.end(), corr[j].begin(), corr[j].end());
+          terms[ncm + j] = {c.small + corr_off[j], corr[j].size()};
+        }
+        HIPCHK(c.upload(c.small, flat.data(), flat.size() * sizeof(Fr)));
+        HIPCHK(lincomb_multi(gbufs.data(), (int)P, n, terms.data(), (int)nt, coef.data(), st));
+        HIPCHK(kate_division_multi(gbufs.data(), super_pts.data() + p0, (int)P, n, c.hx, c.scr, st, p0 > 0));
+      }
+    } else {
+      const size_t cap = sl.hi1 - sl.lo + 1;
+      HIPCHK(c.slab_pk->slab_buf.ensure(np * cap));
+      auto gbuf = [&](size_t i) { return c.slab_pk->slab_buf.p + i * cap - sl.lo; };
+      HIPCHK(hipMemsetAsync(c.hx + sl.lo, 0, (sl.hi1 - sl.lo) * sizeof(Fr), st));
+      for (size_t pi = 0; pi < np; pi++) {
+        const Fr& p = super_pts[pi];
+        Fr* gp = gbuf(pi);
+        const size_t ncorr = alpha_of(p);
+        corr_stage.emplace_back(ncorr, Fr::zero());
+        std::vector<Fr>& corr = corr_stage.back();
+        LinTerms t;
+        bool first = true;
+        for (size_t ci = 0; ci < cm_ids.size(); ci++) {
+          const int r = rs_of[ci];
+          if (!has[r]) continue;
+          if (t.k == LIN_MAXT - 1) {
+            RCCHK(lincomb_range(gp, sl.lo, sl.hi1, t, !first, st));
+            first = false;
+            t.k = 0;
+          }
+          const Fr coef = alpha[r] * ypow[ci];
+          t.p[t.k] = polys[cm_ids[ci]].p;
+          t.len[t.k] = polys[cm_ids[ci]].len;
+          t.coef[t.k] = coef;
+          t.k++;
+          for (size_t j = 0; j < low[ci].size(); j++) corr[j] = corr[j] + coef * low[ci][j];
+        }
+        HIPCHK(c.upload(c.small, corr.data(), corr.size() * sizeof(Fr)));
+        t.p[t.k] = c.small;
+        t.len[t.k] = corr.size();
+        t.coef[t.k] = fr_neg_one();
         t.k++;
-        for (size_t j = 0; j < low[ci].size(); j++) corr[j] = corr[j] + coef * low[ci][j];
-      }
-      HIPCHK(c.upload(c.small, corr.data(), corr.size() * sizeof(Fr)));
-      t.p[t.k] = c.small;
-      t.len[t.k] = corr.size();
-      t.coef[t.k] = fr_neg_one();
-      t.k++;
-      RCCHK(lincomb_range(gp, sl.lo, sl.hi1, t, !first, st));
-      if (!slabs) HIPCHK(kate_division(c.nx, n, p, c.hx, c.scr, st, true));
-    }
-    if (slabs) {
+        RCCHK(lincomb_range(gp, sl.lo, sl.hi1, t, !first, st));
+      }
       std::vector<Fr> carry;
       RCCHK(slab_carries(c, super_pts, [&](size_t i) { return gbuf(i); }, &carry));
       Fr halo = Fr::zero();
@@ -297,17 +342,11 @@
   }
   mark(c, "shplonk h");
   const Fr u = tr.squeeze();
-  Fr z0 = Fr::one();
+  Fr z0 = Fr::one(), c0 = Fr::zero(), zt = Fr::one();
+  std::vector<LinTerm> lterms;
+  std::vector<Fr> lcoef;
   {
-    Fr vpow = Fr::one(), c0 = Fr::zero();
-    LinTerms t;
-    bool first = true;
-    auto flush = [&]() -> int {
-      RCCHK(lincomb_range(c.lx, sl.lo, sl.hi1, t, !first, st));
-      first = false;
-      t.k = 0;
-      return H2G_OK;
-    };
+    Fr vpow = Fr::one();
     for (size_t r = 0; r < rs_rep.size(); r++) {
       const std::vector<Fr>& pts = cm_pts[rs_rep[r]];
       Fr zi = Fr::one();
@@ -317,19 +356,32 @@
       Fr ypow = Fr::one();
       for (size_t ci = 0; ci < cm_ids.size(); ci++) {
         if (rs_of[ci] != (int)r) continue;
-        if (t.k == LIN_MAXT - 2) RCCHK(flush());
         const Fr coef = ypow * zi * vpow;
-        t.p[t.k] = polys[cm_ids[ci]].p;
-        t.len[t.k] = polys[cm_ids[ci]].len;
-        t.coef[t.k] = coef;
-        t.k++;
+        lterms.push_back({polys[cm_ids[ci]].p, polys[cm_ids[ci]].len});
+        lcoef.push_back(coef);
         c0 = c0 - coef * eval_host(low[ci], u);
         ypow = ypow * sy;
       }
       vpow = vpow * v;
     }
-    Fr zt = Fr::one();
     for (auto& sp : super_pts) zt = (u - sp) * zt;
+  }
+  if (slabs) {
+    LinTerms t;
+    bool first = true;
+    auto flush = [&]() -> int {
+      RCCHK(lincomb_range(c.lx, sl.lo, sl.hi1, t, !first, st));
+      first = false;
+      t.k = 0;
+      return H2G_OK;
+    };
+    for (size_t i = 0; i < lterms.size(); i++) {
+      if (t.k == LIN_MAXT - 2) RCCHK(flush());
+      t.p[t.k] = lterms[i].p;
+      t.len[t.k] = lterms[i].len;
+      t.coef[t.k] = lcoef[i];
+      t.k++;
+    }
     c0_stage = c0;
     HIPCHK(c.upload(c.small, &c0_stage, sizeof(Fr)));
     t.p[t.k] = c.small;
@@ -341,8 +393,6 @@
     t.coef[t.k] = Fr::zero() - zt;
     t.k++;
     RCCHK(flush());
-  }
-  if (slabs) {
     std::vector<Fr> carry;
     const std::vector<Fr> pts{u};
     RCCHK(slab_carries(c, pts, [&](size_t) { return c.lx; }, &carry));
@@ -353,8 +403,17 @@
       HIPCHK(poly_binop(POLY_SCALE, c.q1 + sl.lo, nullptr, inv(z0), c.q1 + sl.lo, hq - sl.lo, st));
     }
   } else {
+    const Fr z0i = inv(z0);
+    for (Fr& cf : lcoef) cf = cf * z0i;
+    c0_stage = c0 * z0i;
+    HIPCHK(c.upload(c.small, &c0_stage, sizeof(Fr)));
+    lterms.push_back({c.small, 1});
+    lcoef.push_back(Fr::one());
+    lterms.push_back({c.hx, n});
+    lcoef.push_back(Fr::zero() - zt * z0i);
+    Fr* const out = c.lx;
+    HIPCHK(lincomb_multi(&out, 1, n, lterms.data(), (int)lterms.size(), lcoef.data(), st));
     HIPCHK(kate_division(c.lx, n, u, c.q1, c.scr, st));
-    HIPCHK(poly_binop(POLY_SCALE, c.q1, nullptr, inv(z0), c.q1, n - 1, st));
   }
   {
     G1Affine cm;
diff --git a/yet-another-halo2-fork_amd/csrc/prover_kernels.h b/yet-another-halo2-fork_amd/csrc/prover_kernels.h
--- a/yet-another-halo2-fork_amd/csrc/prover_kernels.h
+++ b/yet-another-halo2-fork_amd/csrc/prover_kernels.h
@@ -196,6 +196,16 @@
   int k = 0;
 };
 hipError_t lincomb(Fr* out, uint64_t n, const LinTerms& t, bool accumulate, hipStream_t st);
+static constexpr int LIN_MAXO = 4;
+static constexpr int LINM_MAXT = 20;
+struct LinTerm {
+  const Fr* p;
+  uint64_t len;
+};
+hipError_t lincomb_multi(Fr* const* out, int nout, uint64_t n, const LinTerm* terms, int nterms, const Fr* coef,
+                         hipStream_t st);
+hipError_t kate_division_multi(const Fr* const* a, const Fr* b, int np, uint64_t len, Fr* q, Fr* scratch,
+                               hipStream_t st, bool accumulate = false, int force_s = 0);
 hipError_t scale_by_dev(Fr* out, const Fr* a, uint64_t n, const Fr* scalar, hipStream_t st);
 
 hipError_t sigma_from_mapping(Fr* sigma, const uint32_t* map_col, const uint32_t* map_row, size_t n,
diff --git a/yet-another-halo2-fork_amd/csrc/prover_kernels.hip b/yet-another-halo2-fork_amd/csrc/prover_kernels.hip
--- a/yet-another-halo2-fork_amd/csrc/prover_kernels.hip
+++ b/yet-another-halo2-fork_amd/csrc/prover_kernels.hip
@@ -750,7 +750,7 @@
   if (t == 0) tile_val[blockIdx.x] = sh[0];
 }
 
-__global__ void __launch_bounds__(KD_T) kate_phase2(Fr* __restrict__ tile_val, uint64_t ntiles, Fr B) {
+__device__ __forceinline__ void kate_phase2_block(Fr* __restrict__ tile_val, uint64_t ntiles, const Fr& B) {
   __shared__ Fr shv[KD_T], shw[KD_T];
   const uint64_t per = (ntiles + KD_T - 1) / KD_T;
   const uint64_t lo = (uint64_t)threadIdx.x * per;
@@ -768,6 +768,9 @@
     tile_val[i] = carry;
     carry = v + B * carry;
   }
+}
+__global__ void __launch_bounds__(KD_T) kate_phase2(Fr* __restrict__ tile_val, uint64_t ntiles, Fr B) {
+  kate_phase2_block(tile_val, ntiles, B);
 }
 
 template <int KD_S, bool ACC>
@@ -833,6 +836,17 @@
   return S;
 }
 
+static KatePow kate_pow(const Fr& b, int S) {
+  KatePow pw;
+  Fr x = b;
+  for (int i = 1; i < S; i <<= 1) x = x * x;
+  for (int l = 0; l <= KD_L; l++) {
+    pw.p[l] = x;
+    x = x * x;
+  }
+  return pw;
+}
+
 hipError_t kate_division(const Fr* a, uint64_t len, const Fr& b, Fr* q, Fr* scratch, hipStream_t st,
                          bool accumulate, int force_s) {
   if (len < 2) return hipSuccess;
@@ -841,13 +855,7 @@
   const int S = force_s ? force_s : kate_tile_s(M);
   const uint64_t tile_len = (uint64_t)KD_T * S;
   const uint64_t nt = (M + tile_len - 1) / tile_len;
-  KatePow pw;
-  Fr x = b;
-  for (int i = 1; i < S; i <<= 1) x = x * x;
-  for (int l = 0; l <= KD_L; l++) {
-    pw.p[l] = x;
-    x = x * x;
-  }
+  const KatePow pw = kate_pow(b, S);
   Fr* tile = scratch;
   Fr* thr = scratch + nt + 1;
   const F29 b29 = storage_to_f29<FrParams>(b);
@@ -856,6 +864,160 @@
     case 16: kate_launch<16>(a, M, b, b29, pw, tile, thr, q, nt, st, accumulate); break;
     case 32: kate_launch<32>(a, M, b, b29, pw, tile, thr, q, nt, st, accumulate); break;
     default: kate_launch<64>(a, M, b, b29, pw, tile, thr, q, nt, st, accumulate); break;
+  }
+  return hipGetLastError();
+}
+
+template <int I, int N, class F>
+__device__ __forceinline__ void sfor_p(F&& f) {
+  if constexpr (I < N) {
+    f(std::integral_constant<int, I>{});
+    sfor_p<I + 1, N>(f);
+  }
+}
+struct KateMulti {
+  const Fr* a1[LIN_MAXO];
+  F29 b29[LIN_MAXO];
+  KatePow pw[LIN_MAXO];
+};
+struct KateTileB {
+  Fr B[LIN_MAXO];
+};
+
+template <int KD_S, int P>
+__global__ void __launch_bounds__(KD_T) kate_phase1_multi(KateMulti A, uint64_t M, Fr* __restrict__ scratch,
+                                                          uint64_t stride, uint64_t nt) {
+  __shared__ Fr sh[KD_T];
+  const int t = threadIdx.x;
+  const uint64_t lo = blockIdx.x * (uint64_t)(KD_T * KD_S) + (uint64_t)t * KD_S;
+  F29 a29[P];
+  sfor_p<0, P>([&](auto p) { a29[p] = F29{}; });
+#pragma unroll 4
+  for (int i = KD_S - 1; i >= 0; i--) {
+    const uint64_t j = lo + i;
+    sfor_p<0, P>([&](auto p) {
+      a29[p] = add29(mul29<FrParams>(a29[p], A.b29[p]), j < M ? raw29(ldf(A.a1[p] + j)) : F29{});
+    });
+  }
+  sfor_p<0, P>([&](auto p) {
+    Fr* tile_val = scratch + p * stride;
+    Fr* thr_val = tile_val + nt + 1;
+    const Fr acc = f29_to_storage(a29[p]);
+    stf(thr_val + blockIdx.x * (uint64_t)KD_T + t, acc);
+    sh[t] = acc;
+    __syncthreads();
+#pragma unroll
+    for (int l = 0; l < KD_L; l++) {
+      const int s = 1 << l;
+      if ((t & (2 * s - 1)) == 0) sh[t] = sh[t] + A.pw[p].p[l] * sh[t + s];
+      __syncthreads();
+    }
+    if (t == 0) tile_val[blockIdx.x] = sh[0];
+    __syncthreads();
+  });
+}
+
+__global__ void __launch_bounds__(KD_T) kate_phase2_multi(Fr* __restrict__ scratch, uint64_t stride, uint64_t ntiles,
+                                                          KateTileB tb) {
+  kate_phase2_block(scratch + blockIdx.x * stride, ntiles, tb.B[blockIdx.x]);
+}
+
+template <int KD_S, int P>
+__global__ void __launch_bounds__(KD_T) kate_phase3_multi(KateMulti A, uint64_t M, const Fr* __restrict__ scratch,
+                                                          uint64_t stride, uint64_t nt, Fr* __restrict__ q,
+                                                          int acc_in) {
+  __shared__ Fr sh[KD_T];
+  __shared__ KateStage stg;
+  const int t = threadIdx.x;
+  const uint64_t g = blockIdx.x * (uint64_t)KD_T + t;
+  F29 cur[P];
+  sfor_p<0, P>([&](auto p) {
+    const Fr* tile_carry = scratch + p * stride;
+    const Fr* thr_val = tile_carry + nt + 1;
+    Fr x = t + 1 < KD_T ? ldf(thr_val + g + 1) : tile_carry[blockIdx.x];
+#pragma unroll
+    for (int l = 0; l < KD_L; l++) {
+      const int s = 1 << l;
+      sh[t] = x;
+      __syncthreads();
+      if (t + s < KD_T) x = x + A.pw[p].p[l] * sh[t + s];
+      __syncthreads();
+    }
+    cur[p] = raw29(x);
+  });
+  const uint64_t tile0 = blockIdx.x * (uint64_t)(KD_T * KD_S);
+  for (int c = KD_S / KD_SUB - 1; c >= 0; c--) {
+    F29 sum[KD_SUB];
+#pragma unroll
+    for (int i = 0; i < KD_SUB; i++) sum[i] = F29{};
+    if (acc_in) {
+      __syncthreads();
+      kate_stage_load<KD_S>(stg, q, tile0, M, c);
+      __syncthreads();
+#pragma unroll
+      for (int i = 0; i < KD_SUB; i++) sum[i] = raw29(kate_stage_get(stg, t, i));
+    }
+    sfor_p<0, P>([&](auto p) {
+      __syncthreads();
+      kate_stage_load<KD_S>(stg, A.a1[p], tile0, M, c);
+      __syncthreads();
+#pragma unroll
+      for (int i = KD_SUB - 1; i >= 0; i--) {
+        cur[p] = add29(raw29(kate_stage_get(stg, t, i)), mul29<FrParams>(cur[p], A.b29[p]));
+        sum[i] = norm29(add29(sum[i], cur[p]));
+      }
+    });
+#pragma unroll
+    for (int i = 0; i < KD_SUB; i++) kate_stage_put(stg, t, i, f29_to_storage(sum[i]));
+    __syncthreads();
+    kate_stage_store<KD_S>(stg, q, tile0, M, c);
+  }
+}
+
+template <int S, int P>
+static void kate_multi_launch(const KateMulti& A, const KateTileB& tb, uint64_t M, Fr* scratch, uint64_t stride,
+                              uint64_t nt, Fr* q, hipStream_t st, bool accumulate) {
+  hipLaunchKernelGGL((kate_phase1_multi<S, P>), dim3((unsigned)nt), dim3(KD_T), 0, st, A, M, scratch, stride, nt);
+  hipLaunchKernelGGL(kate_phase2_multi, dim3(P), dim3(KD_T), 0, st, scratch, stride, nt, tb);
+  hipLaunchKernelGGL((kate_phase3_multi<S, P>), dim3((unsigned)nt), dim3(KD_T), 0, st, A, M, (const Fr*)scratch, stride,
+                     nt, q, accumulate ? 1 : 0);
+}
+template <int S>
+static void kate_multi_launch_p(int np, const KateMulti& A, const KateTileB& tb, uint64_t M, Fr* scratch,
+                                uint64_t stride, uint64_t nt, Fr* q, hipStream_t st, bool accumulate) {
+  static_assert(LIN_MAXO == 4, "one arm per dividend count");
+  switch (np) {
+    case 1: kate_multi_launch<S, 1>(A, tb, M, scratch, stride, nt, q, st, accumulate); break;
+    case 2: kate_multi_launch<S, 2>(A, tb, M, scratch, stride, nt, q, st, accumulate); break;
+    case 3: kate_multi_launch<S, 3>(A, tb, M, scratch, stride, nt, q, st, accumulate); break;
+    default: kate_multi_launch<S, 4>(A, tb, M, scratch, stride, nt, q, st, accumulate); break;
+  }
+}
+
+hipError_t kate_division_multi(const Fr* const* a, const Fr* b, int np, uint64_t len, Fr* q, Fr* scratch,
+                               hipStream_t st, bool accumulate, int force_s) {
+  if (np < 1 || np > LIN_MAXO) return hipErrorInvalidValue;
+  if (force_s && force_s != 8 && force_s != 16 && force_s != 32 && force_s != 64) return hipErrorInvalidValue;
+  if (len < 2) return hipSuccess;
+  const uint64_t M = len - 1;
+  const int S = force_s ? force_s : kate_tile_s(M);
+  const uint64_t tile_len = (uint64_t)KD_T * S;
+  const uint64_t nt = (M + tile_len - 1) / tile_len;
+  const uint64_t stride = kate_scratch_len(len);
+  KateMulti A;
+  KateTileB tb;
+  for (int p = 0; p < LIN_MAXO; p++) {
+    const int s = p < np ? p : 0;
+    A.a1[p] = a[s] + 1;
+    A.b29[p] = storage_to_f29<FrParams>(b[s]);
+    A.pw[p] = kate_pow(b[s], S);
+    tb.B[p] = A.pw[p].p[KD_L];
+  }
+  switch (S) {
+    case 8: kate_multi_launch_p<8>(np, A, tb, M, scratch, stride, nt, q, st, accumulate); break;
+    case 16: kate_multi_launch_p<16>(np, A, tb, M, scratch, stride, nt, q, st, accumulate); break;
+    case 32: kate_multi_launch_p<32>(np, A, tb, M, scratch, stride, nt, q, st, accumulate); break;
+    default: kate_multi_launch_p<64>(np, A, tb, M, scratch, stride, nt, q, st, accumulate); break;
   }
   return hipGetLastError();
 }
@@ -896,6 +1058,81 @@
   return hipGetLastError();
 }
 
+struct LinMulti29 {
+  Fr* out[LIN_MAXO];
+  const Fr* p[LINM_MAXT];
+  uint64_t len[LINM_MAXT];
+  F29 coef[LIN_MAXO][LINM_MAXT];
+  uint32_t nz[LIN_MAXO];
+  int k = 0;
+};
+static_assert(LINM_MAXT <= 32 && LINM_MAXT % 2 == 0, "nz holds a bit per term; terms go in pairs");
+static_assert(sizeof(LinMulti29) <= 3800, "the term table travels as a kernel argument");
+template <int NO>
+__global__ void __launch_bounds__(KT) lincomb_multi_kernel(uint64_t n, LinMulti29 t, int acc_in) {
+  for (uint64_t i = blockIdx.x * (uint64_t)blockDim.x + threadIdx.x; i < n; i += (uint64_t)gridDim.x * blockDim.x) {
+    F29 acc[NO];
+    sfor_p<0, NO>([&](auto o) { acc[o] = acc_in ? raw29(ldf(t.out[o] + i)) : F29{}; });
+    for (int k = 0; k < t.k; k += 2) {
+      const F29 a = i < t.len[k] ? raw29(ldf(t.p[k] + i)) : F29{};
+      const F29 b = k + 1 < t.k && i < t.len[k + 1] ? raw29(ldf(t.p[k + 1] + i)) : F29{};
+      sfor_p<0, NO>([&](auto o) {
+        const uint32_t m = (t.nz[o] >> k) & 3u;
+        if (m == 3u) acc[o] = norm29(add29(acc[o], mul29x2<FrParams>(a, t.coef[o][k], b, t.coef[o][k + 1])));
+        else if (m == 1u) acc[o] = norm29(add29(acc[o], mul29<FrParams>(a, t.coef[o][k])));
+        else if (m == 2u) acc[o] = norm29(add29(acc[o], mul29<FrParams>(b, t.coef[o][k + 1])));
+      });
+    }
+    sfor_p<0, NO>([&](auto o) {
+      stf(t.out[o] + i, pack29<FrParams>(sub_m_if_ge29<FrParams>(reduce29<FrParams>(norm29(acc[o])))));
+    });
+  }
+}
+
+hipError_t lincomb_multi(Fr* const* out, int nout, uint64_t n, const LinTerm* terms, int nterms, const Fr* coef,
+                         hipStream_t st) {
+  if (n == 0) return hipSuccess;
+  static_assert(LIN_MAXO == 4, "one arm per output count");
+  const Fr zero = Fr::zero();
+  for (int o0 = 0; o0 < nout; o0 += LIN_MAXO) {
+    const int no = std::min(LIN_MAXO, nout - o0);
+    LinMulti29 t{};
+    for (int o = 0; o < LIN_MAXO; o++) t.out[o] = out[o0 + (o < no ? o : 0)], t.nz[o] = 0;
+    bool first = true;
+    auto flush = [&]() {
+      for (int k = t.k; k < LINM_MAXT; k++) t.p[k] = nullptr, t.len[k] = 0;
+      const dim3 grid(grid_1d(n)), block(KT);
+      const int acc = first ? 0 : 1;
+      switch (no) {
+        case 1: hipLaunchKernelGGL(lincomb_multi_kernel<1>, grid, block, 0, st, n, t, acc); break;
+        case 2: hipLaunchKernelGGL(lincomb_multi_kernel<2>, grid, block, 0, st, n, t, acc); break;
+        case 3: hipLaunchKernelGGL(lincomb_multi_kernel<3>, grid, block, 0, st, n, t, acc); break;
+        default: hipLaunchKernelGGL(lincomb_multi_kernel<4>, grid, block, 0, st, n, t, acc); break;
+      }
+      first = false;
+      t.k = 0;
+      for (int o = 0; o < LIN_MAXO; o++) t.nz[o] = 0;
+    };
+    for (int k = 0; k < nterms; k++) {
+      uint32_t used = 0;
+      for (int o = 0; o < no; o++)
+        if (!(coef[(size_t)(o0 + o) * nterms + k] == zero)) used |= 1u << o;
+      if (!used || terms[k].len == 0) continue;
+      if (t.k == LINM_MAXT) flush();
+      t.p[t.k] = terms[k].p;
+      t.len[t.k] = terms[k].len;
+      for (int o = 0; o < no; o++) {
+        if (!(used >> o & 1)) continue;
+        t.coef[o][t.k] = storage_to_f29<FrParams>(coef[(size_t)(o0 + o) * nterms + k]);
+        t.nz[o] |= 1u << t.k;
+      }
+      t.k++;
+    }
+    if (t.k || first) flush();
+  }
+  return hipGetLastError();
+}
+
 __global__ void __launch_bounds__(KT) scale_dev_kernel(Fr* __restrict__ out, const Fr* __restrict__ a, uint64_t n,
                                                        const Fr* __restrict__ s) {
   const Fr c = ldf(s);
diff --git a/yet-another-halo2-fork_amd/h2g.py b/yet-another-halo2-fork_amd/h2g.py
--- a/yet-another-halo2-fork_amd/h2g.py
+++ b/yet-another-halo2-fork_amd/h2g.py
@@ -177,6 +177,9 @@
     "h2g_kate_division_dev": ([VP, SZ, U64P, VP, VP], I32),
     "h2g_debug_kate_division_dev": ([VP, SZ, U64P, VP, I32, I32, VP], I32),
     "h2g_debug_kate_tile_s": ([SZ, ctypes.POINTER(I32)], I32),
+    "h2g_debug_lincomb_multi_limits": ([ctypes.POINTER(I32), ctypes.POINTER(I32)], I32),
+    "h2g_debug_lincomb_multi_dev": ([ctypes.POINTER(VP), U64P, I32, U64P, ctypes.POINTER(VP), I32, SZ, VP], I32),
+    "h2g_debug_kate_division_multi_dev": ([ctypes.POINTER(VP), U64P, I32, SZ, VP, I32, I32, VP], I32),
     "h2g_multiopen_prove": ([U64, I32, U64, VP, SZ, VP, SZ], I32),
     "h2g_multiopen_verify": ([VP, I32, U64, U64P, SZ, VP, SZ, ctypes.POINTER(ctypes.c_int32), U64P], I32),
     "h2g_pairing_check_batch": ([VP, U64P, SZ, ctypes.POINTER(ctypes.c_int32)], I32),
@@ -1527,6 +1530,29 @@
     return s.value
 
 
+def debug_lincomb_multi_limits():
+    o, t = I32(0), I32(0)
+    check(lib().h2g_debug_lincomb_multi_limits(ctypes.byref(o), ctypes.byref(t)))
+    return o.value, t.value
+
+
+def debug_lincomb_multi_dev(d_terms, lens, coef, d_outs, n, stream=None):
+    nt, no = len(d_terms), len(d_outs)
+    cf = np.ascontiguousarray(coef, dtype=np.uint64).reshape(no * nt * 4)
+    ln = np.ascontiguousarray(lens, dtype=np.uint64).reshape(nt)
+    terms = (VP * max(nt, 1))(*[VP(p) for p in d_terms])
+    outs = (VP * no)(*[VP(p) for p in d_outs])
+    check(lib().h2g_debug_lincomb_multi_dev(terms, p64(ln) if nt else None, nt, p64(cf) if nt else None, outs, no, n,
+                                            VP(stream) if stream else None))
+
+
+def debug_kate_division_multi_dev(d_as, points, n, d_q, accumulate=False, tile_s=0, stream=None):
+    pts = np.ascontiguousarray(points, dtype=np.uint64).reshape(len(d_as) * 4)
+    arr = (VP * len(d_as))(*[VP(p) for p in d_as])
+    check(lib().h2g_debug_kate_division_multi_dev(arr, p64(pts), len(d_as), n, VP(d_q), int(bool(accumulate)), tile_s,
+                                                  VP(stream) if stream else None))
+
+
 def msm_segmented(bases, scalars, seg_off, index=None):
     bs = np.ascontiguousarray(bases, dtype=np.uint64).reshape(-1, 8)
     sc = np.ascontiguousarray(scalars, dtype=np.uint64).reshape(-1, 4)
```

After: 0.07260, median of 6. No clear change (-0.5%).
